# KerkDovan/univer-ocr

Measured on AMD Instinct MI355X. Metric: document-images/sec (fwd+bwd) on 256x512 synthetic pages, higher is better.
Workload: dtype f32; 1 GPU; BASELINE configs[2]: my_model train step (fwd+loss+bwd+L2+SGD) of Monochrome+Paragraph+Line on (32,256,512,1) pages and Char on (32,32,64,1) line strips per GPU; batch_per_gpu=32, global_batch=32, optimizer=sgd, parallelism=dp1, h2d_inclusive=False, input_grads=True, hip_graphs=True, pipelined_lanes=True, hw_queues=4

## Files before the change

### include/univer_hip.h

```cpp
#ifndef UNIVER_HIP_H
#define UNIVER_HIP_H

#include <stddef.h>
#include <stdint.h>

#ifdef __cplusplus
extern "C" {
#endif

#define UOCR_ABI_VERSION 4

typedef struct uocr_ctx uocr_ctx;

enum { UOCR_F32 = 0, UOCR_F64 = 1, UOCR_F16 = 2 };
#define UOCR_F16_SCALED(k) (UOCR_F16 | ((k) << 8))
#define UOCR_DTYPE_BASE(dtype) ((dtype) & 0xff)
#define UOCR_DTYPE_GRAD_SCALE_LOG2(dtype) (((dtype) >> 8) & 0xff)
enum { UOCR_ACT_NONE = 0, UOCR_ACT_RELU = 1, UOCR_ACT_LEAKY = 2, UOCR_ACT_SIGMOID = 3 };
enum { UOCR_LOSS_DICE = 0, UOCR_LOSS_JACCARD = 1 };
enum {
    UOCR_OK = 0,
    UOCR_ERR_ARG = -1,
    UOCR_ERR_DTYPE = -2,
    UOCR_ERR_HIP = -3,
    UOCR_ERR_WORKSPACE = -4,
    UOCR_ERR_UNSUPPORTED = -5,
    UOCR_ERR_RCCL = -6
};

int uocr_abi_version(void);
int uocr_ctx_create(int device, size_t workspace_bytes, uocr_ctx** out);
int uocr_ctx_create_cu_mask(int device, size_t workspace_bytes, const uint32_t* cu_mask, int mask_words, uocr_ctx** out);
int uocr_ctx_destroy(uocr_ctx* ctx);
int uocr_ctx_set_stream(uocr_ctx* ctx, void* hip_stream);
void* uocr_ctx_get_stream(uocr_ctx* ctx);
int uocr_ctx_set_option(uocr_ctx* ctx, const char* key, int value);
int uocr_ctx_last_split(uocr_ctx* ctx, int* blocks, long long* items);
int uocr_ctx_last_gemm(uocr_ctx* ctx, int* bm, int* gm, int* gn, int* nsplit);
int uocr_ctx_last_gemm_group(uocr_ctx* ctx, int* problems, int* split_problems);
int uocr_ctx_last_pair(uocr_ctx* ctx, int* kernel, int* g, int* mode, int* pf, int* nw, int* blocks_x, int* bands,
                       int* band_h);
int uocr_ctx_reserve_workspace(uocr_ctx* ctx, size_t bytes);
const char* uocr_last_error(uocr_ctx* ctx);
int uocr_malloc(uocr_ctx* ctx, size_t bytes, void** out);
int uocr_free(uocr_ctx* ctx, void* ptr);
int uocr_memset_zero(uocr_ctx* ctx, void* ptr, size_t bytes);
int uocr_h2d(uocr_ctx* ctx, void* dst, const void* src_host, size_t bytes);
int uocr_d2h_sync(uocr_ctx* ctx, void* dst_host, const void* src, size_t bytes);
int uocr_d2d(uocr_ctx* ctx, void* dst, const void* src, size_t bytes);
int uocr_stream_sync(uocr_ctx* ctx);
int uocr_event_create(void** out_event);
int uocr_event_destroy(void* event);
int uocr_event_record(uocr_ctx* ctx, void* event);
int uocr_stream_wait_event(uocr_ctx* ctx, void* event);
int uocr_event_elapsed_ms_sync(void* start, void* stop, float* out_ms);
int uocr_event_synchronize(void* event);
int uocr_graph_begin_capture(uocr_ctx* ctx);
int uocr_graph_end_capture(uocr_ctx* ctx, void** out_graph_exec);
int uocr_graph_launch(uocr_ctx* ctx, void* graph_exec);
int uocr_graph_destroy(void* graph_exec);
int uocr_ctx_set_loss_snapshot(uocr_ctx* ctx, const double* slots, int count, double* ring, int ring_len,
                               unsigned* counter);
int uocr_wgrad_defer_begin(uocr_ctx* ctx);
int uocr_wgrad_defer_flush(uocr_ctx* ctx, int keep_open);
int uocr_device_info(uocr_ctx* ctx, char* name_out, size_t name_cap, int* cu_count, size_t* hbm_bytes);

int uocr_conv2d_fwd(uocr_ctx* ctx, int dtype, const void* x, const void* w, const void* b, void* y,
                    int n, int h, int wd, int cin, int cout, int kh, int kw, int sh, int sw,
                    int ph, int pw, int oh, int ow, double pad_value, int use_bias,
                    int act, double act_alpha);
int uocr_conv2d_bwd_data(uocr_ctx* ctx, int dtype, const void* dy, const void* w, void* dx,
                         int n, int h, int wd, int cin, int cout, int kh, int kw, int sh, int sw,
                         int ph, int pw, int oh, int ow,
                         const void* x_act, int act, double act_alpha);
int uocr_conv2d_bwd_weight(uocr_ctx* ctx, int dtype, const void* x, const void* dy, void* dw, void* db,
                           int n, int h, int wd, int cin, int cout, int kh, int kw, int sh, int sw,
                           int ph, int pw, int oh, int ow, double pad_value, int use_bias,
                           int accumulate);

int uocr_conv_pair_fwd(uocr_ctx* ctx, int dtype, const void* x, const void* w1, const void* b1,
                       const void* w2, const void* b2, void* y, int n, int h, int wd, int cmid,
                       double pad_value1, int use_bias1, int use_bias2, double alpha1, int act2);
int uocr_conv_pair_bwd(uocr_ctx* ctx, int dtype, const void* x, const void* y, const void* dy,
                       const void* w1, const void* b1, const void* w2, void* dw1, void* db1, void* dw2,
                       void* db2, void* dx, int n, int h, int wd, int cmid, double pad_value1,
                       int use_bias1, int use_bias2, double alpha1, int act2, int accumulate);

int uocr_upconv2x_fwd(uocr_ctx* ctx, int dtype, const void* x_low, const void* w, const void* b, void* y,
                      int n, int hl, int wl, int cin, int cout, int kh, int kw, int ph, int pw,
                      int use_bias, int act, double act_alpha, void* weff);
int uocr_upconv2x_bwd_data(uocr_ctx* ctx, int dtype, const void* dy, const void* w, void* dx_low,
                           int n, int hl, int wl, int cin, int cout, int kh, int kw, int ph, int pw,
                           const void* x_act, int act, double act_alpha, const void* weff);
int uocr_upconv2x_bwd_weight(uocr_ctx* ctx, int dtype, const void* x_low, const void* dy, void* dw, void* db,
                             int n, int hl, int wl, int cin, int cout, int kh, int kw, int ph, int pw,
                             int use_bias, int accumulate);

int uocr_maxpool2d_fwd(uocr_ctx* ctx, int dtype, const void* x, void* y, uint8_t* mask,
                       int n, int h, int wd, int c, int kh, int kw, int sh, int sw, int ph, int pw,
                       int oh, int ow);
int uocr_maxpool2d_bwd(uocr_ctx* ctx, int dtype, const void* dy, const uint8_t* mask, void* dx,
                       int n, int h, int wd, int c, int kh, int kw, int sh, int sw, int ph, int pw,
                       int oh, int ow);

int uocr_upsample2d_fwd(uocr_ctx* ctx, int dtype, const void* x, void* y,
                        int n, int h, int wd, int c, int sy, int sx);
int uocr_upsample2d_bwd(uocr_ctx* ctx, int dtype, const void* dy, void* dx,
                        int n, int h, int wd, int c, int sy, int sx);

int uocr_act_fwd(uocr_ctx* ctx, int dtype, int kind, double alpha, const void* x, void* y, size_t count);
int uocr_act_bwd(uocr_ctx* ctx, int dtype, int kind, double alpha, const void* x, const void* dy,
                 void* dx, size_t count);

int uocr_act_bwd_from_output(uocr_ctx* ctx, int dtype, int kind, double alpha, const void* y, const void* dy,
                             void* dx, size_t count);

int uocr_dense_fwd(uocr_ctx* ctx, int dtype, const void* x, const void* w, void* y,
                   int m, int n_in, int n_out);
int uocr_dense_bwd(uocr_ctx* ctx, int dtype, const void* x, const void* w, const void* dy,
                   void* dx, void* dw, int m, int n_in, int n_out, int accumulate);
int uocr_dense_fwd_act(uocr_ctx* ctx, int dtype, const void* x, const void* w, void* y,
                       int m, int n_in, int n_out, int act, double act_alpha);
int uocr_dense_bwd_act(uocr_ctx* ctx, int dtype, const void* x, const void* w, const void* dy,
                       void* dx, void* dw, int m, int n_in, int n_out, int accumulate,
                       int x_act, double x_act_alpha);

int uocr_fixed_width_fwd(uocr_ctx* ctx, int dtype, const void* x, void* y,
                         int n, int h, int wd, int c, int width);
int uocr_fixed_width_bwd(uocr_ctx* ctx, int dtype, const void* dy, void* dx,
                         int n, int h, int wd, int c, int width);

int uocr_copy_2d(uocr_ctx* ctx, int dtype, void* dst, size_t dst_ld, const void* src, size_t src_ld,
                 size_t rows, size_t cols);
int uocr_add(uocr_ctx* ctx, int dtype, const void* a, const void* b, void* out, size_t count);
int uocr_axpy(uocr_ctx* ctx, int dtype, double alpha, const void* x, void* y, size_t count);
int uocr_scale(uocr_ctx* ctx, int dtype, double alpha, void* x, size_t count);
int uocr_fill(uocr_ctx* ctx, int dtype, void* x, double value, size_t count);
int uocr_convert(uocr_ctx* ctx, int src_dtype, const void* src, int dst_dtype, void* dst, size_t count);
int uocr_u8_to_float(uocr_ctx* ctx, int dtype, const uint8_t* src, void* dst, double scale, size_t count);

int uocr_seg_loss(uocr_ctx* ctx, int dtype, int kind , const void* pred,
                  const void* gt, void* grad , double* loss_out,
                  int n, int hw, int c, int out_act);
int uocr_softmax_ce(uocr_ctx* ctx, int dtype, const void* pred, const void* gt, void* grad ,
                    double* loss_out, int m, int c);
int uocr_sigmoid_ce(uocr_ctx* ctx, int dtype, const void* pred, const void* gt, void* grad ,
                    double* loss_out, int m, size_t count);

int uocr_l2_reg(uocr_ctx* ctx, int dtype, const void* w, void* grad, size_t count, double strength,
                double* loss_out, int accumulate_loss);
int uocr_l1_reg(uocr_ctx* ctx, int dtype, const void* w, void* grad, size_t count, double strength,
                double* loss_out, int accumulate_loss);

int uocr_adam_step(uocr_ctx* ctx, int dtype, void* w, const void* g, void* v, void* a, size_t count,
                   double lr, double beta1, double beta2, double eps);
int uocr_momentum_step(uocr_ctx* ctx, int dtype, void* w, const void* g, void* v, size_t count,
                       double lr, double momentum);
int uocr_momentum_step_fused(uocr_ctx* ctx, int dtype, void* w, void* g, void* v, size_t count, double lr,
                             double momentum, int nranges, const long long* lo, const long long* hi,
                             const int* kind, const double* strength, double* reg_loss_out, int zero_grad,
                             const double* hyper_dev);
int uocr_adam_step_fused(uocr_ctx* ctx, int dtype, void* w, void* g, void* v, void* a, size_t count, double lr,
                         double beta1, double beta2, double eps, int nranges, const long long* lo,
                         const long long* hi, const int* kind, const double* strength, double* reg_loss_out,
                         int zero_grad, const double* hyper_dev );
int uocr_rmsprop_step(uocr_ctx* ctx, int dtype, void* w, const void* g, void* a, size_t count,
                      double lr, double rho, double eps);
int uocr_has_nan(uocr_ctx* ctx, int dtype, const void* x, size_t count, int32_t* flag_out);

#define UOCR_DP_UNIQUE_ID_BYTES 128
int uocr_dp_get_unique_id(void* out_bytes );
int uocr_dp_init(uocr_ctx* ctx, int rank, int world, const void* unique_id_bytes);
int uocr_dp_info(uocr_ctx* ctx, int* rank, int* world );
int uocr_dp_allreduce_sum(uocr_ctx* ctx, void* buf, size_t count, int dtype);
int uocr_dp_broadcast(uocr_ctx* ctx, void* buf, size_t count, int dtype, int root);
int uocr_dp_finalize(uocr_ctx* ctx);
int uocr_dp_version(int* out_version);

#ifdef __cplusplus
}
#endif
#endif
```

### univer-ocr_amd/csrc/conv_up.hip

```cpp
#include "up_phase.h"
#include "finish_group.h"
#include "conv_dims.h"

namespace {

using f32x4 = __attribute__((ext_vector_type(4))) float;

constexpr int CH = 4;
constexpr int RH = 16, RW = 32;
constexpr int XH = RH + 2, XW = RW + 2;
constexpr int XPLANE = 624;
constexpr int NWEFF = 9 * CH * 16;

__device__ __forceinline__ f32x4 mfma(float a, float b, f32x4 c) {
    return __builtin_amdgcn_mfma_f32_16x16x4f32(a, b, c, 0, 0, 0);
}

__device__ __forceinline__ float act_apply(float v, int act, float alpha) {
    switch (act) {
        case UOCR_ACT_RELU: return v * (v >= 0.f ? 1.f : 0.f);
        case UOCR_ACT_LEAKY: return v * ((v >= 0.f ? 1.f : 0.f) + alpha * (v < 0.f ? 1.f : 0.f));
        case UOCR_ACT_SIGMOID: return 1.f / (1.f + expf(-v));
        default: return v;
    }
}

__host__ __device__ __forceinline__ void tap_group(int phase, int mi, int& lo, int& hi) {
    if (phase == 0) {
        lo = 2 * mi;
        hi = mi == 2 ? 5 : 2 * mi + 2;
    } else {
        lo = mi == 0 ? 0 : 2 * mi - 1;
        hi = mi == 0 ? 1 : 2 * mi + 1;
    }
}

__global__ __launch_bounds__(256) void upconv_weff_kernel(const float* __restrict__ w, float* __restrict__ weff) {
    for (int i = threadIdx.x; i < NWEFF; i += blockDim.x) {
        const int o = i & 3, phase = (i >> 2) & 3, c = (i >> 4) & 3, m = i >> 6;
        int ylo, yhi, xlo, xhi;
        tap_group(phase >> 1, m / 3, ylo, yhi);
        tap_group(phase & 1, m % 3, xlo, xhi);
        float s = 0.f;
        for (int ky = ylo; ky < yhi; ++ky)
            for (int kx = xlo; kx < xhi; ++kx) s += w[((ky * 5 + kx) * CH + c) * CH + o];
        weff[i] = s;
    }
}

template <typename TA>
__device__ __forceinline__ void stage_planar(float* __restrict__ xs, const TA* __restrict__ xb, int ry, int rx,
                                             int hl, int wl, int tid) {
    if constexpr (sizeof(TA) == 4) {
        stage_batched<XH * XW, 256, 3, float4>(
            tid,
            [&](int i, bool& inside) {
                const int r = i / XW, c = i - r * XW;
                const int gy = ry - 1 + r, gx = rx - 1 + c;
                inside = gy >= 0 && gy < hl && gx >= 0 && gx < wl;
                return reinterpret_cast<const float4*>(xb + ((size_t)min(max(gy, 0), hl - 1) * wl + min(max(gx, 0), wl - 1)) * CH);
            },
            [&](int i, float4 v, bool inside) {
                if (!inside) v = make_float4(0.f, 0.f, 0.f, 0.f);
                xs[i] = v.x;
                xs[XPLANE + i] = v.y;
                xs[2 * XPLANE + i] = v.z;
                xs[3 * XPLANE + i] = v.w;
            });
        return;
    }
    for (int i = tid; i < XH * XW; i += 256) {
        const int r = i / XW, c = i - r * XW;
        const int gy = ry - 1 + r, gx = rx - 1 + c;
        float4 v = make_float4(0.f, 0.f, 0.f, 0.f);
        if (gy >= 0 && gy < hl && gx >= 0 && gx < wl) v = ld4(xb + ((size_t)gy * wl + gx) * CH);
        xs[i] = v.x;
        xs[XPLANE + i] = v.y;
        xs[2 * XPLANE + i] = v.z;
        xs[3 * XPLANE + i] = v.w;
    }
}

template <typename TA>
__global__ __launch_bounds__(256) void upconv_fwd_kernel(const TA* __restrict__ xl, const float* __restrict__ w,
                                                         const float* __restrict__ bias, TA* __restrict__ y,
                                                         int hl, int wl, int rows_per_block, int use_bias, int act,
                                                         float alpha, float* __restrict__ weff_out) {
    __shared__ float xs[CH * XPLANE];
    const int tid = threadIdx.x, lane = tid & 63, wv = tid >> 6, n = lane & 15, kq = lane >> 4;
    if (weff_out && blockIdx.x == 0 && blockIdx.y == 0 && blockIdx.z == 0) {
        for (int i = tid; i < NWEFF; i += 256) {
            const int o = i & 3, phase = (i >> 2) & 3, c = (i >> 4) & 3, m = i >> 6;
            int ylo, yhi, xlo, xhi;
            tap_group(phase >> 1, m / 3, ylo, yhi);
            tap_group(phase & 1, m % 3, xlo, xhi);
            float s = 0.f;
            for (int ky = ylo; ky < yhi; ++ky)
                for (int kx = xlo; kx < xhi; ++kx) s += w[((ky * 5 + kx) * CH + c) * CH + o];
            weff_out[i] = s;
        }
    }
    const int rx = blockIdx.x * RW;
    const int row_begin = blockIdx.y * rows_per_block, row_end = min(hl, row_begin + rows_per_block);
    const TA* xb = xl + (size_t)blockIdx.z * hl * wl * CH;
    const int W = 2 * wl;
    TA* yb = y + (size_t)blockIdx.z * (2 * hl) * W * CH;
    float wa[9];
#pragma unroll
    for (int t = 0; t < 9; ++t) {
        int ylo, yhi, xlo, xhi;
        tap_group(n >> 3, t / 3, ylo, yhi);
        tap_group((n >> 2) & 1, t % 3, xlo, xhi);
        float s = 0.f;
        for (int ky = ylo; ky < yhi; ++ky)
            for (int kx = xlo; kx < xhi; ++kx) s += w[((ky * 5 + kx) * CH + kq) * CH + (n & 3)];
        wa[t] = s;
    }
    f32x4 b4 = {0.f, 0.f, 0.f, 0.f};
    if (use_bias) b4 = f32x4{bias[0], bias[1], bias[2], bias[3]};
    for (int ry = row_begin; ry < row_end; ry += RH) {
        __syncthreads();
        stage_planar(xs, xb, ry, rx, hl, wl, tid);
        __syncthreads();
#pragma unroll 2
        for (int k = 0; k < 8; ++k) {
            const int gi = wv * 8 + k, r = gi >> 1, c0 = (gi & 1) * 16;
            const float* xr = xs + kq * XPLANE + r * XW + c0 + n;
            f32x4 acc = b4;
#pragma unroll
            for (int t = 0; t < 9; ++t) acc = mfma(wa[t], xr[(t / 3) * XW + t % 3], acc);
            const int py = ry + r, pxl = rx + c0 + n;
            if (py < row_end && pxl < wl) {
                float4 out;
                out.x = act_apply(acc[0], act, alpha);
                out.y = act_apply(acc[1], act, alpha);
                out.z = act_apply(acc[2], act, alpha);
                out.w = act_apply(acc[3], act, alpha);
                st4(yb + ((size_t)(2 * py + (kq >> 1)) * W + 2 * pxl + (kq & 1)) * CH, out);
            }
        }
    }
}

template <typename TA>
__global__ __launch_bounds__(256) void upconv_wgrad_kernel(const TA* __restrict__ xl, const TA* __restrict__ dy,
                                                           float* __restrict__ partial, int hl, int wl,
                                                           int rows_per_block) {
    __shared__ float xs[CH * XPLANE];
    __shared__ float red[4][48][16];
    __shared__ float reddb[4][64];
    const int tid = threadIdx.x, lane = tid & 63, wv = tid >> 6, n = lane & 15, kq = lane >> 4;
    const int rx = blockIdx.x * RW;
    const int row_begin = blockIdx.y * rows_per_block, row_end = min(hl, row_begin + rows_per_block);
    const TA* xb = xl + (size_t)blockIdx.z * hl * wl * CH;
    const int W = 2 * wl;
    const TA* gb = dy + (size_t)blockIdx.z * (2 * hl) * W * CH;
    int aoff[3];
    bool aok[3];
#pragma unroll
    for (int j = 0; j < 3; ++j) {
        const int K = 16 * j + n;
        aok[j] = K < 36;
        const int Kc = aok[j] ? K : 35, t = Kc >> 2;
        aoff[j] = (Kc & 3) * XPLANE + (t / 3) * XW + t % 3 + kq;
    }
    const int boff = ((n >> 3) * W + ((n >> 2) & 1)) * CH + (n & 3);
    f32x4 acc[3] = {{0.f, 0.f, 0.f, 0.f}, {0.f, 0.f, 0.f, 0.f}, {0.f, 0.f, 0.f, 0.f}};
    float dbacc = 0.f;
    for (int ry = row_begin; ry < row_end; ry += RH) {
        __syncthreads();
        stage_planar(xs, xb, ry, rx, hl, wl, tid);
        __syncthreads();
#pragma unroll 2
        for (int k = 0; k < 8; ++k) {
            const int gi = wv * 8 + k, r = gi >> 1, c0 = (gi & 1) * 16;
            const int py = ry + r;
            const bool row_ok = py < row_end;
            const float* xr = xs + r * XW + c0;
            const TA* gr = gb + ((size_t)(2 * min(py, hl - 1)) * W + 2 * rx) * CH + boff;
#pragma unroll
            for (int i = 0; i < 4; ++i) {
                const int pl = c0 + 4 * i + kq;
                const bool ok = row_ok && rx + pl < wl;
                float g = ld1(gr + (size_t)2 * min(pl, wl - 1 - rx) * CH);
                g = ok ? g : 0.f;
                dbacc += g;
#pragma unroll
                for (int j = 0; j < 3; ++j) {
                    const float xv = xr[4 * i + aoff[j]];
                    acc[j] = mfma(aok[j] ? xv : 0.f, g, acc[j]);
                }
            }
        }
    }
#pragma unroll
    for (int j = 0; j < 3; ++j)
#pragma unroll
        for (int v = 0; v < 4; ++v) red[wv][16 * j + 4 * kq + v][n] = acc[j][v];
    reddb[wv][lane] = dbacc;
    __syncthreads();
    if (tid < 4) {
        float s = 0.f;
        for (int w = 0; w < 4; ++w)
            for (int l = tid; l < 64; l += 4) s += reddb[w][l];
        reddb[0][tid] = s;
    }
    __syncthreads();
    const int blk = (blockIdx.z * gridDim.y + blockIdx.y) * gridDim.x + blockIdx.x;
    up4_write_row(partial + (size_t)blk * UP4_NOUT, [&](int i) {
        if (i >= 576) return reddb[0][i - 576];
        const int K = i >> 4, col = i & 15;
        return red[0][K][col] + red[1][K][col] + red[2][K][col] + red[3][K][col];
    }, tid, 256);
}

__global__ __launch_bounds__(256) void colsum_finish_kernel(const float* __restrict__ partial, int nblocks, int ncols,
                                                            int ndw, float* __restrict__ dw, float* __restrict__ db,
                                                            int use_bias, int accumulate, float unscale) {
    constexpr int FC = 8, NSEG = 32;
    __shared__ double seg[NSEG][FC];
    const int o = threadIdx.x % FC, sg = threadIdx.x / FC, j = blockIdx.x * FC + o;
    double s = 0.0;
    if (j < ncols) {
        const int per = (nblocks + NSEG - 1) / NSEG, b0 = sg * per, b1 = min(nblocks, b0 + per);
        int b = b0;
        for (; b + 8 <= b1; b += 8) {
            float v[8];
#pragma unroll
            for (int k = 0; k < 8; ++k) v[k] = partial[(size_t)(b + k) * ncols + j];
#pragma unroll
            for (int k = 0; k < 8; ++k) s += (double)v[k];
        }
        for (; b < b1; ++b) s += (double)partial[(size_t)b * ncols + j];
    }
    seg[sg][o] = s;
    __syncthreads();
    if (sg != 0 || j >= ncols) return;
#pragma unroll
    for (int k = 1; k < NSEG; ++k) s += seg[k][o];
    float* dst = j < ndw ? dw + j : db + (j - ndw);
    if (j >= ndw && !use_bias) s = 0.0;
    s *= (double)unscale;
    *dst = accumulate ? (float)((double)*dst + s) : (float)s;
}

constexpr int GH = 2 * (RH + 2), GW = 2 * (RW + 2);
template <typename TA>
__global__ __launch_bounds__(256) void upconv_dgrad_kernel(const TA* __restrict__ dy, const float* __restrict__ weff,
                                                           TA* __restrict__ dxl, int hl, int wl,
                                                           const TA* __restrict__ mask_y, int mask_act,
                                                           float mask_alpha) {
    __shared__ float4 gs[GH * GW];
    const int tid = threadIdx.x;
    const int rx = blockIdx.x * RW, ry = blockIdx.y * RH;
    const int H = 2 * hl, W = 2 * wl;
    const TA* gb = dy + (size_t)blockIdx.z * H * W * CH;
    if constexpr (sizeof(TA) == 4) {
        stage_batched<GH * GW, 256, 5, float4>(
            tid,
            [&](int i, bool& inside) {
                const int r = i / GW, c = i - r * GW;
                const int gy = 2 * (ry - 1) + r, gx = 2 * (rx - 1) + c;
                inside = gy >= 0 && gy < H && gx >= 0 && gx < W;
                return reinterpret_cast<const float4*>(gb + ((size_t)min(max(gy, 0), H - 1) * W + min(max(gx, 0), W - 1)) * CH);
            },
            [&](int i, float4 v, bool inside) { gs[i] = inside ? v : make_float4(0.f, 0.f, 0.f, 0.f); });
    } else {
        for (int i = tid; i < GH * GW; i += 256) {
            const int r = i / GW, c = i - r * GW;
            const int gy = 2 * (ry - 1) + r, gx = 2 * (rx - 1) + c;
            float4 v = make_float4(0.f, 0.f, 0.f, 0.f);
            if (gy >= 0 && gy < H && gx >= 0 && gx < W) v = ld4(gb + ((size_t)gy * W + gx) * CH);
            gs[i] = v;
        }
    }
    __syncthreads();
    const int c = tid & 31, r0 = tid >> 5;
    float acc[2][4];
#pragma unroll
    for (int p = 0; p < 2; ++p)
#pragma unroll
        for (int j = 0; j < 4; ++j) acc[p][j] = 0.f;
#pragma unroll 1
    for (int m = 0; m < 9; ++m) {
        const float* wt = weff + m * 64;
        const int my = m / 3 - 1, mx = m % 3 - 1;
#pragma unroll
        for (int p = 0; p < 2; ++p) {
            const int r = r0 + 8 * p;
            const float4* g0 = gs + (2 * (r - my + 1)) * GW + 2 * (c - mx + 1);
            const float4 g[4] = {g0[0], g0[1], g0[GW], g0[GW + 1]};
#pragma unroll
            for (int ch = 0; ch < 4; ++ch)
#pragma unroll
                for (int phase = 0; phase < 4; ++phase) {
                    const float* wv = wt + ch * 16 + phase * 4;
                    acc[p][ch] += wv[0] * g[phase].x + wv[1] * g[phase].y + wv[2] * g[phase].z + wv[3] * g[phase].w;
                }
        }
    }
#pragma unroll
    for (int p = 0; p < 2; ++p) {
        const int qy = ry + r0 + 8 * p, qx = rx + c;
        if (qy >= hl || qx >= wl) continue;
        const size_t off = (((size_t)blockIdx.z * hl + qy) * wl + qx) * CH;
        float4 out = make_float4(acc[p][0], acc[p][1], acc[p][2], acc[p][3]);
        if (mask_act != UOCR_ACT_NONE) {
            const float4 yv = ld4(mask_y + off);
            out.x *= act_grad_from_output<float>(yv.x, mask_act, mask_alpha);
            out.y *= act_grad_from_output<float>(yv.y, mask_act, mask_alpha);
            out.z *= act_grad_from_output<float>(yv.z, mask_act, mask_alpha);
            out.w *= act_grad_from_output<float>(yv.w, mask_act, mask_alpha);
        }
        st4(dxl + off, out);
    }
}

__device__ __forceinline__ void weff1_build(float (&we)[36], const float* __restrict__ w) {
#pragma unroll
    for (int m = 0; m < 9; ++m)
#pragma unroll
        for (int phase = 0; phase < 4; ++phase) {
            int ylo, yhi, xlo, xhi;
            tap_group(phase >> 1, m / 3, ylo, yhi);
            tap_group(phase & 1, m % 3, xlo, xhi);
            float s = 0.f;
            for (int ky = ylo; ky < yhi; ++ky)
                for (int kx = xlo; kx < xhi; ++kx) s += w[ky * 5 + kx];
            we[m * 4 + phase] = s;
        }
}

template <typename TA>
__global__ __launch_bounds__(256) void up1_fwd_kernel(const TA* __restrict__ xl, const float* __restrict__ w,
                                                      const float* __restrict__ bias, TA* __restrict__ y, int hl,
                                                      int wl, int use_bias, int act, float alpha) {
    __shared__ float xs[XH * XW];
    const int tid = threadIdx.x;
    const int rx = blockIdx.x * RW, ry = blockIdx.y * RH;
    const TA* xb = xl + (size_t)blockIdx.z * hl * wl;
    stage_batched<XH * XW, 256, 3, TA>(
        tid,
        [&](int i, bool& inside) {
            const int r = i / XW, c = i - r * XW;
            const int gy = ry - 1 + r, gx = rx - 1 + c;
            inside = gy >= 0 && gy < hl && gx >= 0 && gx < wl;
            return xb + (size_t)min(max(gy, 0), hl - 1) * wl + min(max(gx, 0), wl - 1);
        },
        [&](int i, TA v, bool inside) { xs[i] = inside ? (float)v : 0.f; });
    float we[36];
    weff1_build(we, w);
    const float b0 = use_bias ? bias[0] : 0.f;
    __syncthreads();
    const int c = tid & 31, r0 = tid >> 5;
    const int W = 2 * wl;
    TA* yb = y + (size_t)blockIdx.z * (2 * hl) * W;
#pragma unroll
    for (int p = 0; p < 2; ++p) {
        const int r = r0 + 8 * p, py = ry + r, pxl = rx + c;
        float acc[4] = {b0, b0, b0, b0};
#pragma unroll
        for (int m = 0; m < 9; ++m) {
            const float xv = xs[(r + m / 3) * XW + c + m % 3];
#pragma unroll
            for (int phase = 0; phase < 4; ++phase) acc[phase] += xv * we[m * 4 + phase];
        }
        if (py < hl && pxl < wl) {
            TA* o = yb + (size_t)(2 * py) * W + 2 * pxl;
            st2(o, make_float2(act_apply(acc[0], act, alpha), act_apply(acc[1], act, alpha)));
            st2(o + W, make_float2(act_apply(acc[2], act, alpha), act_apply(acc[3], act, alpha)));
        }
    }
}

template <typename TA>
__global__ __launch_bounds__(256) void up1_dgrad_kernel(const TA* __restrict__ dy, const float* __restrict__ w,
                                                        TA* __restrict__ dxl, int hl, int wl,
                                                        const TA* __restrict__ mask_y, int mask_act,
                                                        float mask_alpha) {
    __shared__ float gs[GH * GW];
    const int tid = threadIdx.x;
    const int rx = blockIdx.x * RW, ry = blockIdx.y * RH;
    const int H = 2 * hl, W = 2 * wl;
    const TA* gb = dy + (size_t)blockIdx.z * H * W;
    stage_batched<GH * GW, 256, 10, TA>(
        tid,
        [&](int i, bool& inside) {
            const int r = i / GW, c = i - r * GW;
            const int gy = 2 * (ry - 1) + r, gx = 2 * (rx - 1) + c;
            inside = gy >= 0 && gy < H && gx >= 0 && gx < W;
            return gb + (size_t)min(max(gy, 0), H - 1) * W + min(max(gx, 0), W - 1);
        },
        [&](int i, TA v, bool inside) { gs[i] = inside ? (float)v : 0.f; });
    float we[36];
    weff1_build(we, w);
    __syncthreads();
    const int c = tid & 31, r0 = tid >> 5;
#pragma unroll
    for (int p = 0; p < 2; ++p) {
        const int r = r0 + 8 * p;
        float acc = 0.f;
#pragma unroll
        for (int m = 0; m < 9; ++m) {
            const int my = m / 3 - 1, mx = m % 3 - 1;
            const float* g0 = gs + (2 * (r - my + 1)) * GW + 2 * (c - mx + 1);
            acc += we[m * 4] * g0[0] + we[m * 4 + 1] * g0[1] + we[m * 4 + 2] * g0[GW] + we[m * 4 + 3] * g0[GW + 1];
        }
        const int qy = ry + r, qx = rx + c;
        if (qy >= hl || qx >= wl) continue;
        const size_t off = ((size_t)blockIdx.z * hl + qy) * wl + qx;
        if (mask_act != UOCR_ACT_NONE) acc *= act_grad_from_output<float>(ld1(mask_y + off), mask_act, mask_alpha);
        st1(dxl + off, acc);
    }
}

template <typename TA>
__global__ __launch_bounds__(256) void up1_wgrad_kernel(const TA* __restrict__ xl, const TA* __restrict__ dy,
                                                        float* __restrict__ partial, int hl, int wl,
                                                        int rows_per_block) {
    __shared__ float xs[XH * XW];
    __shared__ float red[4][37];
    const int tid = threadIdx.x;
    const int rx = blockIdx.x * RW;
    const int row_begin = blockIdx.y * rows_per_block, row_end = min(hl, row_begin + rows_per_block);
    const TA* xb = xl + (size_t)blockIdx.z * hl * wl;
    const int W = 2 * wl;
    const TA* gb = dy + (size_t)blockIdx.z * (2 * hl) * W;
    const int c = tid & 31, r0 = tid >> 5;
    float acc[36], dbacc = 0.f;
#pragma unroll
    for (int i = 0; i < 36; ++i) acc[i] = 0.f;
    for (int ry = row_begin; ry < row_end; ry += RH) {
        __syncthreads();
        stage_batched<XH * XW, 256, 3, TA>(
            tid,
            [&](int i, bool& inside) {
                const int r = i / XW, cc = i - r * XW;
                const int gy = ry - 1 + r, gx = rx - 1 + cc;
                inside = gy >= 0 && gy < hl && gx >= 0 && gx < wl;
                return xb + (size_t)min(max(gy, 0), hl - 1) * wl + min(max(gx, 0), wl - 1);
            },
            [&](int i, TA v, bool inside) { xs[i] = inside ? (float)v : 0.f; });
        __syncthreads();
#pragma unroll
        for (int p = 0; p < 2; ++p) {
            const int r = r0 + 8 * p, py = ry + r, pxl = rx + c;
            if (py >= row_end || pxl >= wl) continue;
            const TA* g0 = gb + (size_t)(2 * py) * W + 2 * pxl;
            const float2 ga = ld2(g0), gbv = ld2(g0 + W);
            const float g[4] = {ga.x, ga.y, gbv.x, gbv.y};
            dbacc += (g[0] + g[1]) + (g[2] + g[3]);
#pragma unroll
            for (int m = 0; m < 9; ++m) {
                const float xv = xs[(r + m / 3) * XW + c + m % 3];
#pragma unroll
                for (int phase = 0; phase < 4; ++phase) acc[m * 4 + phase] += xv * g[phase];
            }
        }
    }
    const int lane = tid & 63, wv = tid >> 6;
#pragma unroll
    for (int i = 0; i < 36; ++i) {
        const float v = wave_reduce_sum(acc[i]);
        if (lane == 0) red[wv][i] = v;
    }
    dbacc = wave_reduce_sum(dbacc);
    if (lane == 0) red[wv][36] = dbacc;
    __syncthreads();
    const int blk = (blockIdx.z * gridDim.y + blockIdx.y) * gridDim.x + blockIdx.x;
    up1_write_row(partial + (size_t)blk * UP1_NOUT, [&](int i) { return red[0][i] + red[1][i] + red[2][i] + red[3][i]; }, tid);
}


int up_rows_per_block(int strips, int hl, int n, unsigned max_blocks = 2048u) {
    int rows = RH;
    while (rows < hl && (size_t)strips * ((hl + rows - 1) / rows) * n > max_blocks) rows += RH;
    return rows;
}

int check_up(uocr_ctx* ctx, int dtype, int n, int hl, int wl, int cin, int cout, int kh, int kw, int ph, int pw) {
    if (UOCR_DTYPE_BASE(dtype) != UOCR_F32 && UOCR_DTYPE_BASE(dtype) != UOCR_F16)
        UOCR_FAIL(ctx, UOCR_ERR_UNSUPPORTED, "upconv2x: float32 / float16 only");
    if (!((cin == CH && cout == CH) || (cin == 1 && cout == 1)) || kh != 5 || kw != 5 || ph != 2 || pw != 2)
        UOCR_FAIL(ctx, UOCR_ERR_UNSUPPORTED,
                  "upconv2x: 5x5 / padding 2 / 4 -> 4 or 1 -> 1 channels only (got %dx%d pad %d,%d %d -> %d)", kh, kw, ph,
                  pw, cin, cout);
    UOCR_REQUIRE(ctx, n > 0 && hl > 0 && wl > 0 && n <= 65535);
    return UOCR_OK;
}

}

extern "C" int uocr_upconv2x_fwd(uocr_ctx* ctx, int dtype, const void* x_low, const void* w, const void* b, void* y,
                                 int n, int hl, int wl, int cin, int cout, int kh, int kw, int ph, int pw,
                                 int use_bias, int act, double act_alpha, void* weff) {
    UOCR_CHECK_CTX(ctx);
    UOCR_REQUIRE(ctx, x_low && w && b && y);
    int rc = check_up(ctx, dtype, n, hl, wl, cin, cout, kh, kw, ph, pw);
    if (rc != UOCR_OK) return rc;
    if (uocr_upconv_h16_eligible(ctx, dtype, cin, cout) && uocr_aligned_act(x_low, dtype) && uocr_aligned_act(y, dtype))
        return uocr_upconv_fwd_h16(ctx, x_low, w, b, y, n, hl, wl, use_bias, act, act_alpha);
    const int strips = (wl + RW - 1) / RW, rows = up_rows_per_block(strips, hl, n, (unsigned)uocr_budget(ctx, 2048));
    if (cin != 1) uocr_note_split(ctx, (long long)strips * ((hl + rows - 1) / rows) * n, (long long)strips * ((hl + RH - 1) / RH) * n);
    UOCR_DISPATCH_TA(ctx, dtype, {
        if (cin == 1)
            hipLaunchKernelGGL((up1_fwd_kernel<TA>), dim3((wl + RW - 1) / RW, (hl + RH - 1) / RH, n), dim3(256), 0,
                               ctx->stream, (const TA*)x_low, (const float*)w, (const float*)b, (TA*)y, hl, wl, use_bias,
                               act, (float)act_alpha);
        else
            hipLaunchKernelGGL((upconv_fwd_kernel<TA>), dim3(strips, (hl + rows - 1) / rows, n), dim3(256), 0,
                               ctx->stream, (const TA*)x_low, (const float*)w, (const float*)b, (TA*)y, hl, wl, rows,
                               use_bias, act, (float)act_alpha, (float*)weff);
    });
    UOCR_LAUNCH_CHECK(ctx);
    return UOCR_OK;
}

extern "C" int uocr_upconv2x_bwd_data(uocr_ctx* ctx, int dtype, const void* dy, const void* w, void* dx_low, int n,
                                      int hl, int wl, int cin, int cout, int kh, int kw, int ph, int pw,
                                      const void* x_act, int act, double act_alpha, const void* weff_in) {
    UOCR_CHECK_CTX(ctx);
    UOCR_REQUIRE(ctx, dy && w && dx_low);
    UOCR_REQUIRE(ctx, act == UOCR_ACT_NONE || x_act != nullptr);
    int rc = check_up(ctx, dtype, n, hl, wl, cin, cout, kh, kw, ph, pw);
    if (rc != UOCR_OK) return rc;
    if (uocr_upconv_h16_eligible(ctx, dtype, cin, cout) && uocr_aligned_act(dy, dtype) &&
        uocr_aligned_act(dx_low, dtype) && (act == UOCR_ACT_NONE || uocr_aligned_act(x_act, dtype)))
        return uocr_upconv_dgrad_h16(ctx, dy, w, dx_low, n, hl, wl, act == UOCR_ACT_NONE ? nullptr : x_act, act, act_alpha);
    if (uocr_upconv_t32_eligible(ctx, dtype, cin, cout) && (reinterpret_cast<uintptr_t>(dy) & 15u) == 0 &&
        (reinterpret_cast<uintptr_t>(dx_low) & 15u) == 0 && (act == UOCR_ACT_NONE || (reinterpret_cast<uintptr_t>(x_act) & 15u) == 0))
        return uocr_upconv_dgrad_t32(ctx, dy, w, dx_low, n, hl, wl, cin, act == UOCR_ACT_NONE ? nullptr : x_act, act, act_alpha);
    const float* weff = (const float*)weff_in;
    if (cin != 1 && !weff) {
        rc = uocr_need_workspace(ctx, NWEFF * sizeof(float));
        if (rc != UOCR_OK) return rc;
        hipLaunchKernelGGL(upconv_weff_kernel, dim3(1), dim3(256), 0, ctx->stream, (const float*)w, (float*)ctx->workspace);
        weff = (const float*)ctx->workspace;
    }
    const dim3 grid((wl + RW - 1) / RW, (hl + RH - 1) / RH, n);
    UOCR_DISPATCH_TA(ctx, dtype, {
        if (cin == 1)
            hipLaunchKernelGGL((up1_dgrad_kernel<TA>), grid, dim3(256), 0, ctx->stream, (const TA*)dy, (const float*)w,
                               (TA*)dx_low, hl, wl, (const TA*)x_act, act, (float)act_alpha);
        else
            hipLaunchKernelGGL((upconv_dgrad_kernel<TA>), grid, dim3(256), 0, ctx->stream, (const TA*)dy,
                               weff, (TA*)dx_low, hl, wl, (const TA*)x_act, act, (float)act_alpha);
    });
    UOCR_LAUNCH_CHECK(ctx);
    return UOCR_OK;
}

extern "C" int uocr_upconv2x_bwd_weight(uocr_ctx* ctx, int dtype, const void* x_low, const void* dy, void* dw, void* db,
                                        int n, int hl, int wl, int cin, int cout, int kh, int kw, int ph, int pw,
                                        int use_bias, int accumulate) {
    UOCR_CHECK_CTX(ctx);
    UOCR_REQUIRE(ctx, x_low && dy && dw && db);
    int rc = check_up(ctx, dtype, n, hl, wl, cin, cout, kh, kw, ph, pw);
    if (rc != UOCR_OK) return rc;
    const float unscale = (float)uocr_grad_unscale(dtype);
    const int ncols = cin == 1 ? UP1_NOUT : UP4_NOUT, ndw = ncols - cin;
    auto finish = [&](const float* partial, int nblocks) -> int {
        FinishDesc fd{};
        fd.kind = FIN_COLS;
        fd.partial = partial;
        fd.nblocks = nblocks;
        fd.ncols = fd.group_cols = ncols;
        fd.row_stride = ncols;
        fd.dw = (float*)dw, fd.db = (float*)db;
        fd.use_bias = use_bias, fd.accumulate = accumulate;
        fd.unscale = unscale;
        fd.p[0] = ndw;
        if (uocr_finish_defer(ctx, fd)) return UOCR_OK;
        hipLaunchKernelGGL(colsum_finish_kernel, dim3((ncols + 7) / 8), dim3(256), 0, ctx->stream, partial, nblocks, ncols,
                           ndw, (float*)dw, (float*)db, use_bias, accumulate, unscale);
        UOCR_LAUNCH_CHECK(ctx);
        return UOCR_OK;
    };
    if (UOCR_DTYPE_BASE(dtype) == UOCR_F16 && ctx->opt_fast && ctx->opt_h16 && uocr_aligned_act(x_low, dtype) &&
        uocr_aligned_act(dy, dtype)) {
        const size_t floats = (size_t)ctx->cu_count * 8 * ncols;
        float* partial = uocr_partial_buffer(ctx, floats * sizeof(float), &rc);
        if (rc != UOCR_OK) return rc;
        int nblocks = 0;
        rc = uocr_upconv_wgrad_h16(ctx, x_low, dy, partial, floats, n, hl, wl, cin, &nblocks);
        if (rc != UOCR_OK) return rc;
        return finish(partial, nblocks);
    }
    const int strips = (wl + RW - 1) / RW, rows = up_rows_per_block(strips, hl, n, (unsigned)uocr_budget(ctx, 1024));
    const int bands = (hl + rows - 1) / rows, nblocks = strips * bands * n;
    uocr_note_split(ctx, nblocks, (long long)strips * ((hl + RH - 1) / RH) * n);
    float* partial = uocr_partial_buffer(ctx, (size_t)nblocks * ncols * sizeof(float), &rc);
    if (rc != UOCR_OK) return rc;
    UOCR_DISPATCH_TA(ctx, dtype, {
        if (cin == 1)
            hipLaunchKernelGGL((up1_wgrad_kernel<TA>), dim3(strips, bands, n), dim3(256), 0, ctx->stream,
                               (const TA*)x_low, (const TA*)dy, partial, hl, wl, rows);
        else
            hipLaunchKernelGGL((upconv_wgrad_kernel<TA>), dim3(strips, bands, n), dim3(256), 0, ctx->stream,
                               (const TA*)x_low, (const TA*)dy, partial, hl, wl, rows);
    });
    UOCR_LAUNCH_CHECK(ctx);
    return finish(partial, nblocks);
}
```

### univer-ocr_amd/csrc/ctx.hip

```cpp
#include <cstdlib>

#include "finish_group.h"
#include "gemm.h"
#include "uocr_common.h"

extern "C" {

int uocr_abi_version(void) { return UOCR_ABI_VERSION; }

int uocr_ctx_create(int device, size_t workspace_bytes, uocr_ctx** out) {
    if (!out || device < 0) return UOCR_ERR_ARG;
    *out = nullptr;
    int count = 0;
    if (hipGetDeviceCount(&count) != hipSuccess || device >= count) return UOCR_ERR_HIP;
    if (hipSetDevice(device) != hipSuccess) return UOCR_ERR_HIP;
    uocr_ctx* ctx = new uocr_ctx();
    ctx->device = device;
    ctx->err[0] = 0;
    ctx->workspace = nullptr;
    ctx->workspace_bytes = 0;
    ctx->sync = nullptr;
    ctx->gemm_defer = nullptr;
    ctx->snap_src = nullptr;
    ctx->snap_count = 0;
    ctx->snap_ring = nullptr;
    ctx->snap_ring_len = 0;
    ctx->snap_counter = nullptr;
    ctx->finish_defer = nullptr;
    ctx->owns_stream = true;
    ctx->opt_mfma = 1;
    ctx->opt_fast = 1;
    ctx->opt_tiled = 1;
    ctx->opt_split = 1024;
    ctx->opt_split_min = 3;
    ctx->opt_bm = 0;
    ctx->opt_h16 = 1;
    ctx->opt_t32 = 2;
    ctx->opt_xcd = 1;
    ctx->opt_pair_band = 0;
    ctx->opt_pair_g = 4;
    ctx->opt_group_blocks = 0;
    ctx->opt_wgrad_bands = 0;
    ctx->opt_max_blocks = 0;
    ctx->split_blocks = 0;
    ctx->split_items = 0;
    ctx->gemm_bm = ctx->gemm_gm = ctx->gemm_gn = ctx->gemm_nsplit = 0;
    ctx->gemm_group_count = ctx->gemm_group_split = 0;
    uocr_note_pair(ctx, 0, 0, 0, 0, 0, 0, 0, 0);
    ctx->opt_h3 = 0;
#ifdef UOCR_EXPERIMENTS
    if (const char* e = getenv("UOCR_H3")) ctx->opt_h3 = atoi(e);
#endif
    ctx->opt_pair_pf = -1;
    if (const char* e = getenv("UOCR_PAIR_PF")) ctx->opt_pair_pf = atoi(e);
    if (const char* e = getenv("UOCR_WGRAD_BANDS")) ctx->opt_wgrad_bands = atoi(e);
    if (hipStreamCreateWithFlags(&ctx->stream, hipStreamNonBlocking) != hipSuccess) {
        delete ctx;
        return UOCR_ERR_HIP;
    }
    hipDeviceProp_t prop;
    ctx->cu_count = 256;
    if (hipGetDeviceProperties(&prop, device) == hipSuccess) ctx->cu_count = prop.multiProcessorCount;
    if (workspace_bytes) {
        if (hipMalloc(&ctx->workspace, workspace_bytes) != hipSuccess) {
            hipStreamDestroy(ctx->stream);
            delete ctx;
            return UOCR_ERR_HIP;
        }
        ctx->workspace_bytes = workspace_bytes;
    }
    if (hipMalloc((void**)&ctx->sync, UOCR_SYNC_WORDS * sizeof(unsigned)) != hipSuccess ||
        hipMemsetAsync(ctx->sync, 0, UOCR_SYNC_WORDS * sizeof(unsigned), ctx->stream) != hipSuccess ||
        hipStreamSynchronize(ctx->stream) != hipSuccess) {
        if (ctx->sync) hipFree(ctx->sync);
        if (ctx->workspace) hipFree(ctx->workspace);
        hipStreamDestroy(ctx->stream);
        delete ctx;
        return UOCR_ERR_HIP;
    }
    *out = ctx;
    return UOCR_OK;
}

int uocr_ctx_create_cu_mask(int device, size_t workspace_bytes, const uint32_t* cu_mask, int mask_words, uocr_ctx** out) {
    if (!out || !cu_mask || mask_words <= 0) return UOCR_ERR_ARG;
    int rc = uocr_ctx_create(device, workspace_bytes, out);
    if (rc != UOCR_OK) return rc;
    uocr_ctx* ctx = *out;
    hipStream_t masked = nullptr;
    if (hipExtStreamCreateWithCUMask(&masked, (uint32_t)mask_words, cu_mask) != hipSuccess) {
        uocr_ctx_destroy(ctx);
        *out = nullptr;
        return UOCR_ERR_HIP;
    }
    hipStreamDestroy(ctx->stream);
    ctx->stream = masked;
    int cus = 0;
    for (int i = 0; i < mask_words; ++i) cus += __builtin_popcount(cu_mask[i]);
    if (cus > 0 && cus < ctx->cu_count) ctx->cu_count = cus;
    return UOCR_OK;
}

int uocr_ctx_destroy(uocr_ctx* ctx) {
    UOCR_CHECK_CTX(ctx);
    hipSetDevice(ctx->device);
    hipStreamSynchronize(ctx->stream);
    if (ctx->workspace) hipFree(ctx->workspace);
    if (ctx->sync) hipFree(ctx->sync);
    uocr_gemm_defer_free(ctx);
    uocr_finish_defer_free(ctx);
    if (ctx->owns_stream) hipStreamDestroy(ctx->stream);
    delete ctx;
    return UOCR_OK;
}

int uocr_ctx_set_stream(uocr_ctx* ctx, void* hip_stream) {
    UOCR_CHECK_CTX(ctx);
    if (ctx->owns_stream) {
        UOCR_HIP(ctx, hipStreamSynchronize(ctx->stream));
        UOCR_HIP(ctx, hipStreamDestroy(ctx->stream));
        ctx->owns_stream = false;
    }
    ctx->stream = (hipStream_t)hip_stream;
    return UOCR_OK;
}

int uocr_ctx_set_option(uocr_ctx* ctx, const char* key, int value) {
    UOCR_CHECK_CTX(ctx);
    UOCR_REQUIRE(ctx, key != nullptr);
    if (!strcmp(key, "mfma")) ctx->opt_mfma = value;
    else if (!strcmp(key, "fast_paths")) ctx->opt_fast = value;
    else if (!strcmp(key, "tiled")) ctx->opt_tiled = value;
    else if (!strcmp(key, "split_blocks")) ctx->opt_split = value;
    else if (!strcmp(key, "split_min")) ctx->opt_split_min = value;
    else if (!strcmp(key, "gemm_bm")) ctx->opt_bm = value;
    else if (!strcmp(key, "xcd_remap")) ctx->opt_xcd = value;
    else if (!strcmp(key, "h16")) ctx->opt_h16 = value;
    else if (!strcmp(key, "t32")) {
        if (value & ~UOCR_T32_BUILT)
            UOCR_FAIL(ctx, UOCR_ERR_UNSUPPORTED, "option t32 = %d asks for kernels this library was built without "
                      "(UOCR_BUILD_EXPERIMENTS=1 ./build.sh)", value);
        ctx->opt_t32 = value;
    }
    else if (!strcmp(key, "pair_band")) ctx->opt_pair_band = value;
    else if (!strcmp(key, "pair_g")) ctx->opt_pair_g = value;
    else if (!strcmp(key, "group_blocks")) ctx->opt_group_blocks = value;
    else if (!strcmp(key, "wgrad_bands") && value >= 0) ctx->opt_wgrad_bands = value;
    else if (!strcmp(key, "max_blocks") && value >= 0) ctx->opt_max_blocks = value;
    else if (!strcmp(key, "h3")) {
#ifndef UOCR_EXPERIMENTS
        if (value) UOCR_FAIL(ctx, UOCR_ERR_UNSUPPORTED, "option h3: this library was built without conv_h3 "
                             "(UOCR_BUILD_EXPERIMENTS=1 ./build.sh)");
#endif
        ctx->opt_h3 = value;
    }
    else if (!strcmp(key, "pair_pf")) ctx->opt_pair_pf = value;
    else UOCR_FAIL(ctx, UOCR_ERR_ARG, "unknown option '%s'", key);
    return UOCR_OK;
}

int uocr_ctx_last_split(uocr_ctx* ctx, int* blocks, long long* items) {
    UOCR_CHECK_CTX(ctx);
    UOCR_REQUIRE(ctx, blocks && items);
    *blocks = ctx->split_blocks;
    *items = ctx->split_items;
    return UOCR_OK;
}

int uocr_ctx_last_gemm(uocr_ctx* ctx, int* bm, int* gm, int* gn, int* nsplit) {
    UOCR_CHECK_CTX(ctx);
    UOCR_REQUIRE(ctx, bm && gm && gn && nsplit);
    *bm = ctx->gemm_bm;
    *gm = ctx->gemm_gm;
    *gn = ctx->gemm_gn;
    *nsplit = ctx->gemm_nsplit;
    return UOCR_OK;
}

int uocr_ctx_last_gemm_group(uocr_ctx* ctx, int* problems, int* split_problems) {
    UOCR_CHECK_CTX(ctx);
    UOCR_REQUIRE(ctx, problems && split_problems);
    *problems = ctx->gemm_group_count;
    *split_problems = ctx->gemm_group_split;
    return UOCR_OK;
}

int uocr_ctx_last_pair(uocr_ctx* ctx, int* kernel, int* g, int* mode, int* pf, int* nw, int* blocks_x, int* bands,
                       int* band_h) {
    UOCR_CHECK_CTX(ctx);
    UOCR_REQUIRE(ctx, kernel && g && mode && pf && nw && blocks_x && bands && band_h);
    *kernel = ctx->pair_kernel;
    *g = ctx->pair_g;
    *mode = ctx->pair_mode;
    *pf = ctx->pair_pf;
    *nw = ctx->pair_nw;
    *blocks_x = ctx->pair_blocks_x;
    *bands = ctx->pair_bands;
    *band_h = ctx->pair_band_h;
    return UOCR_OK;
}

void* uocr_ctx_get_stream(uocr_ctx* ctx) { return ctx ? (void*)ctx->stream : nullptr; }

int uocr_ctx_reserve_workspace(uocr_ctx* ctx, size_t bytes) {
    UOCR_CHECK_CTX(ctx);
    if (bytes <= ctx->workspace_bytes) return UOCR_OK;
    UOCR_HIP(ctx, hipSetDevice(ctx->device));
    UOCR_HIP(ctx, hipStreamSynchronize(ctx->stream));
    if (ctx->workspace) UOCR_HIP(ctx, hipFree(ctx->workspace));
    ctx->workspace = nullptr;
    ctx->workspace_bytes = 0;
    UOCR_HIP(ctx, hipMalloc(&ctx->workspace, bytes));
    ctx->workspace_bytes = bytes;
    return UOCR_OK;
}

const char* uocr_last_error(uocr_ctx* ctx) { return ctx ? ctx->err : "null context"; }

int uocr_malloc(uocr_ctx* ctx, size_t bytes, void** out) {
    UOCR_CHECK_CTX(ctx);
    UOCR_REQUIRE(ctx, out != nullptr);
    UOCR_HIP(ctx, hipSetDevice(ctx->device));
    UOCR_HIP(ctx, hipMalloc(out, bytes ? bytes : 1));
    return UOCR_OK;
}

int uocr_free(uocr_ctx* ctx, void* ptr) {
    UOCR_CHECK_CTX(ctx);
    if (ptr) UOCR_HIP(ctx, hipFree(ptr));
    return UOCR_OK;
}

int uocr_memset_zero(uocr_ctx* ctx, void* ptr, size_t bytes) {
    UOCR_CHECK_CTX(ctx);
    if (!bytes) return UOCR_OK;
    UOCR_REQUIRE(ctx, ptr != nullptr);
    UOCR_HIP(ctx, hipMemsetAsync(ptr, 0, bytes, ctx->stream));
    return UOCR_OK;
}

int uocr_h2d(uocr_ctx* ctx, void* dst, const void* src_host, size_t bytes) {
    UOCR_CHECK_CTX(ctx);
    if (!bytes) return UOCR_OK;
    UOCR_REQUIRE(ctx, dst && src_host);
    UOCR_HIP(ctx, hipMemcpyAsync(dst, src_host, bytes, hipMemcpyHostToDevice, ctx->stream));
    return UOCR_OK;
}

int uocr_d2h_sync(uocr_ctx* ctx, void* dst_host, const void* src, size_t bytes) {
    UOCR_CHECK_CTX(ctx);
    if (!bytes) return UOCR_OK;
    UOCR_REQUIRE(ctx, dst_host && src);
    UOCR_HIP(ctx, hipMemcpyAsync(dst_host, src, bytes, hipMemcpyDeviceToHost, ctx->stream));
    UOCR_HIP(ctx, hipStreamSynchronize(ctx->stream));
    return UOCR_OK;
}

int uocr_d2d(uocr_ctx* ctx, void* dst, const void* src, size_t bytes) {
    UOCR_CHECK_CTX(ctx);
    if (!bytes) return UOCR_OK;
    UOCR_REQUIRE(ctx, dst && src);
    UOCR_HIP(ctx, hipMemcpyAsync(dst, src, bytes, hipMemcpyDeviceToDevice, ctx->stream));
    return UOCR_OK;
}

int uocr_stream_sync(uocr_ctx* ctx) {
    UOCR_CHECK_CTX(ctx);
    UOCR_HIP(ctx, hipStreamSynchronize(ctx->stream));
    return UOCR_OK;
}

int uocr_event_create(void** out_event) {
    if (!out_event) return UOCR_ERR_ARG;
    hipEvent_t ev;
    if (hipEventCreate(&ev) != hipSuccess) return UOCR_ERR_HIP;
    *out_event = (void*)ev;
    return UOCR_OK;
}

int uocr_event_destroy(void* event) {
    if (!event) return UOCR_ERR_ARG;
    return hipEventDestroy((hipEvent_t)event) == hipSuccess ? UOCR_OK : UOCR_ERR_HIP;
}

int uocr_event_record(uocr_ctx* ctx, void* event) {
    UOCR_CHECK_CTX(ctx);
    UOCR_REQUIRE(ctx, event != nullptr);
    UOCR_HIP(ctx, hipEventRecord((hipEvent_t)event, ctx->stream));
    return UOCR_OK;
}

int uocr_stream_wait_event(uocr_ctx* ctx, void* event) {
    UOCR_CHECK_CTX(ctx);
    UOCR_REQUIRE(ctx, event != nullptr);
    UOCR_HIP(ctx, hipStreamWaitEvent(ctx->stream, (hipEvent_t)event, 0));
    return UOCR_OK;
}

int uocr_event_elapsed_ms_sync(void* start, void* stop, float* out_ms) {
    if (!start || !stop || !out_ms) return UOCR_ERR_ARG;
    if (hipEventSynchronize((hipEvent_t)stop) != hipSuccess) return UOCR_ERR_HIP;
    return hipEventElapsedTime(out_ms, (hipEvent_t)start, (hipEvent_t)stop) == hipSuccess ? UOCR_OK
                                                                                           : UOCR_ERR_HIP;
}

int uocr_event_synchronize(void* event) {
    if (!event) return UOCR_ERR_ARG;
    return hipEventSynchronize((hipEvent_t)event) == hipSuccess ? UOCR_OK : UOCR_ERR_HIP;
}

int uocr_graph_begin_capture(uocr_ctx* ctx) {
    UOCR_CHECK_CTX(ctx);
    UOCR_HIP(ctx, hipStreamBeginCapture(ctx->stream, hipStreamCaptureModeRelaxed));
    return UOCR_OK;
}

int uocr_graph_end_capture(uocr_ctx* ctx, void** out_graph_exec) {
    UOCR_CHECK_CTX(ctx);
    UOCR_REQUIRE(ctx, out_graph_exec != nullptr);
    *out_graph_exec = nullptr;
    hipGraph_t graph = nullptr;
    UOCR_HIP(ctx, hipStreamEndCapture(ctx->stream, &graph));
    hipGraphExec_t exec = nullptr;
    const hipError_t e = hipGraphInstantiate(&exec, graph, nullptr, nullptr, 0);
    hipGraphDestroy(graph);
    if (e != hipSuccess) UOCR_FAIL(ctx, UOCR_ERR_HIP, "hipGraphInstantiate failed: %s", hipGetErrorString(e));
    *out_graph_exec = (void*)exec;
    return UOCR_OK;
}

int uocr_graph_launch(uocr_ctx* ctx, void* graph_exec) {
    UOCR_CHECK_CTX(ctx);
    UOCR_REQUIRE(ctx, graph_exec != nullptr);
    UOCR_HIP(ctx, hipGraphLaunch((hipGraphExec_t)graph_exec, ctx->stream));
    return UOCR_OK;
}

int uocr_graph_destroy(void* graph_exec) {
    if (!graph_exec) return UOCR_ERR_ARG;
    return hipGraphExecDestroy((hipGraphExec_t)graph_exec) == hipSuccess ? UOCR_OK : UOCR_ERR_HIP;
}

int uocr_device_info(uocr_ctx* ctx, char* name_out, size_t name_cap, int* cu_count, size_t* hbm_bytes) {
    UOCR_CHECK_CTX(ctx);
    hipDeviceProp_t prop;
    UOCR_HIP(ctx, hipGetDeviceProperties(&prop, ctx->device));
    if (name_out && name_cap) {
        strncpy(name_out, prop.name, name_cap - 1);
        name_out[name_cap - 1] = 0;
    }
    if (cu_count) *cu_count = prop.multiProcessorCount;
    if (hbm_bytes) *hbm_bytes = prop.totalGlobalMem;
    return UOCR_OK;
}

}
```

### univer-ocr_amd/csrc/uocr_common.h

```cpp
#pragma once
#include <hip/hip_runtime.h>
#include <stdint.h>
#include <stdio.h>
#include <string.h>

#include "univer_hip.h"

struct uocr_ctx {
    int device;
    hipStream_t stream;
    bool owns_stream;
    void* workspace;
    size_t workspace_bytes;
    const double* snap_src;
    int snap_count;
    double* snap_ring;
    int snap_ring_len;
    unsigned* snap_counter;
    void* gemm_defer;
    void* finish_defer;
    unsigned* sync;
    int cu_count;
    int opt_mfma;
    int opt_fast;
    int opt_tiled;
    int opt_split;
    int opt_split_min;
    int opt_xcd;
    int opt_bm;
    int opt_h16;
    int opt_t32;
    int opt_pair_band;
    int opt_pair_pf;
    int opt_h3;
    int opt_group_blocks;
    int opt_wgrad_bands;
    int opt_pair_g;
    int opt_max_blocks;
    int split_blocks;
    long long split_items;
    int gemm_bm, gemm_gm, gemm_gn, gemm_nsplit;
    int gemm_group_count, gemm_group_split;
    int pair_kernel, pair_g, pair_mode, pair_pf;
    int pair_nw, pair_blocks_x, pair_bands, pair_band_h;
    char err[512];
};

constexpr int UOCR_SYNC_WORDS = 1 << 18;
#ifdef UOCR_EXPERIMENTS
constexpr int UOCR_T32_BUILT = 255;
#else
constexpr int UOCR_T32_BUILT = 2;
#endif

#define UOCR_FAIL(ctx, code, ...)                                   \
    do {                                                            \
        if (ctx) snprintf((ctx)->err, sizeof((ctx)->err), __VA_ARGS__); \
        return (code);                                              \
    } while (0)

#define UOCR_HIP(ctx, call)                                                              \
    do {                                                                                 \
        hipError_t e_ = (call);                                                          \
        if (e_ != hipSuccess)                                                            \
            UOCR_FAIL(ctx, UOCR_ERR_HIP, "%s failed: %s (%s:%d)", #call, hipGetErrorString(e_), \
                      __FILE__, __LINE__);                                               \
    } while (0)

#define UOCR_LAUNCH_CHECK(ctx)                                                           \
    do {                                                                                 \
        hipError_t e_ = hipGetLastError();                                               \
        if (e_ != hipSuccess)                                                            \
            UOCR_FAIL(ctx, UOCR_ERR_HIP, "kernel launch failed: %s (%s:%d)", hipGetErrorString(e_), \
                      __FILE__, __LINE__);                                               \
    } while (0)

#define UOCR_REQUIRE(ctx, cond)                                                          \
    do {                                                                                 \
        if (!(cond)) UOCR_FAIL(ctx, UOCR_ERR_ARG, "bad argument: %s (%s:%d)", #cond, __FILE__, __LINE__); \
    } while (0)

#define UOCR_CHECK_CTX(ctx) \
    do {                    \
        if (!(ctx)) return UOCR_ERR_ARG; \
    } while (0)

#define UOCR_DISPATCH(ctx, dtype, ...)                                   \
    do {                                                                 \
        if ((dtype) == UOCR_F32) { using T = float; __VA_ARGS__; }       \
        else if ((dtype) == UOCR_F64) { using T = double; __VA_ARGS__; } \
        else UOCR_FAIL(ctx, UOCR_ERR_DTYPE, "unknown dtype %d", (int)(dtype)); \
    } while (0)

#define UOCR_DISPATCH_ACT(ctx, dtype, ...)                                                        \
    do {                                                                                          \
        const int base_ = UOCR_DTYPE_BASE(dtype);                                                 \
        if (base_ == UOCR_F32) { using TS = float; using T = float; __VA_ARGS__; }                \
        else if (base_ == UOCR_F64) { using TS = double; using T = double; __VA_ARGS__; }         \
        else if (base_ == UOCR_F16) { using TS = _Float16; using T = float; __VA_ARGS__; }        \
        else UOCR_FAIL(ctx, UOCR_ERR_DTYPE, "unknown dtype %d", (int)(dtype));                    \
    } while (0)

#define UOCR_DISPATCH_STORAGE(ctx, dtype, ...)                                                    \
    do {                                                                                          \
        const int base_ = UOCR_DTYPE_BASE(dtype);                                                 \
        if (base_ == UOCR_F32) { using T = float; __VA_ARGS__; }                                  \
        else if (base_ == UOCR_F64) { using T = double; __VA_ARGS__; }                            \
        else if (base_ == UOCR_F16) { using T = _Float16; __VA_ARGS__; }                          \
        else UOCR_FAIL(ctx, UOCR_ERR_DTYPE, "unknown dtype %d", (int)(dtype));                    \
    } while (0)

static inline double uocr_grad_scale(int dtype) {
    return UOCR_DTYPE_BASE(dtype) == UOCR_F16 ? (double)(1u << (UOCR_DTYPE_GRAD_SCALE_LOG2(dtype) & 31)) : 1.0;
}
static inline double uocr_grad_unscale(int dtype) { return 1.0 / uocr_grad_scale(dtype); }

static inline int uocr_need_workspace(uocr_ctx* ctx, size_t bytes) {
    if (bytes > ctx->workspace_bytes)
        UOCR_FAIL(ctx, UOCR_ERR_WORKSPACE, "workspace too small: need %zu bytes, have %zu", bytes,
                  ctx->workspace_bytes);
    return UOCR_OK;
}

static inline unsigned uocr_blocks_for(size_t items, unsigned per_block, unsigned cap) {
    size_t b = (items + per_block - 1) / per_block;
    if (b < 1) b = 1;
    if (b > cap) b = cap;
    return (unsigned)b;
}

static inline long uocr_budget(const uocr_ctx* ctx, long budget) {
    return ctx->opt_max_blocks > 0 && ctx->opt_max_blocks < budget ? ctx->opt_max_blocks : budget;
}
static inline void uocr_note_split(uocr_ctx* ctx, long long blocks, long long items) {
    ctx->split_blocks = (int)blocks;
    ctx->split_items = items;
}

static inline void uocr_note_pair(uocr_ctx* ctx, int kernel, int g, int mode, int pf, int nw, int blocks_x, int bands,
                                  int band_h) {
    ctx->pair_kernel = kernel, ctx->pair_g = g, ctx->pair_mode = mode, ctx->pair_pf = pf;
    ctx->pair_nw = nw, ctx->pair_blocks_x = blocks_x, ctx->pair_bands = bands, ctx->pair_band_h = band_h;
}

constexpr unsigned UOCR_MAX_GRID = 2048;
constexpr int UOCR_WAVE = 64;

template <typename T>
__device__ __forceinline__ T wave_reduce_sum(T v) {
#pragma unroll
    for (int off = 32; off > 0; off >>= 1) v += __shfl_down(v, off, 64);
    return v;
}

template <typename T>
__device__ __forceinline__ T wave_reduce_max(T v) {
#pragma unroll
    for (int off = 32; off > 0; off >>= 1) {
        T o = __shfl_down(v, off, 64);
        v = o > v ? o : v;
    }
    return v;
}

__device__ __forceinline__ double block_reduce_sum(double v, double* smem ) {
    const int lane = threadIdx.x & 63, wid = threadIdx.x >> 6;
    v = wave_reduce_sum(v);
    __syncthreads();
    if (lane == 0) smem[wid] = v;
    __syncthreads();
    const int nw = (blockDim.x + 63) >> 6;
    v = (threadIdx.x < (unsigned)nw) ? smem[threadIdx.x] : 0.0;
    if (wid == 0) v = wave_reduce_sum(v);
    return v;
}

__device__ __forceinline__ void pub_store(double* p, double v) {
    __hip_atomic_store(p, v, __ATOMIC_RELAXED, __HIP_MEMORY_SCOPE_AGENT);
}
__device__ __forceinline__ double pub_load(const double* p) {
    return __hip_atomic_load(p, __ATOMIC_RELAXED, __HIP_MEMORY_SCOPE_AGENT);
}
__device__ __forceinline__ unsigned sync_arrive(unsigned* c) {
    asm volatile("s_waitcnt vmcnt(0)" ::: "memory");
    return __hip_atomic_fetch_add(c, 1u, __ATOMIC_RELAXED, __HIP_MEMORY_SCOPE_AGENT);
}
__device__ __forceinline__ unsigned sync_peek(unsigned* c) {
    return __hip_atomic_load(c, __ATOMIC_RELAXED, __HIP_MEMORY_SCOPE_AGENT);
}
__device__ __forceinline__ void sync_clear(unsigned* c) {
    __hip_atomic_store(c, 0u, __ATOMIC_RELAXED, __HIP_MEMORY_SCOPE_AGENT);
}
__device__ __forceinline__ void last_block_sum(unsigned* counter, double* partial, double mine, int count, double scale,
                                               double* out, double* smem ) {
    if (threadIdx.x == 0) {
        pub_store(partial + blockIdx.x, mine);
        const unsigned t = sync_arrive(counter);
        smem[16] = t == gridDim.x - 1 ? 1.0 : 0.0;
    }
    __syncthreads();
    if (smem[16] == 0.0) return;
    double acc = 0.0;
    if (count <= 4 * (int)blockDim.x) {
        double t[4];
#pragma unroll
        for (int k = 0; k < 4; ++k) {
            const int i = threadIdx.x + k * blockDim.x;
            t[k] = i < count ? pub_load(partial + i) : 0.0;
        }
#pragma unroll
        for (int k = 0; k < 4; ++k) acc += t[k];
    } else {
        for (int i = threadIdx.x; i < count; i += blockDim.x) acc += pub_load(partial + i);
    }
    acc = block_reduce_sum(acc, smem);
    if (threadIdx.x == 0) {
        *out = scale * acc;
        sync_clear(counter);
    }
}

using uocr_h2 = __attribute__((ext_vector_type(2))) _Float16;
using uocr_h4 = __attribute__((ext_vector_type(4))) _Float16;

__device__ __forceinline__ float ld1(const float* p) { return *p; }
__device__ __forceinline__ float ld1(const _Float16* p) { return (float)*p; }
__device__ __forceinline__ float2 ld2(const float* p) { return *reinterpret_cast<const float2*>(p); }
__device__ __forceinline__ float2 ld2(const _Float16* p) {
    const uocr_h2 v = *reinterpret_cast<const uocr_h2*>(p);
    return make_float2((float)v.x, (float)v.y);
}
__device__ __forceinline__ float4 ld4(const float* p) { return *reinterpret_cast<const float4*>(p); }
__device__ __forceinline__ float4 ld4(const _Float16* p) {
    const uocr_h4 v = *reinterpret_cast<const uocr_h4*>(p);
    return make_float4((float)v.x, (float)v.y, (float)v.z, (float)v.w);
}
__device__ __forceinline__ void st1(float* p, float v) { *p = v; }
__device__ __forceinline__ void st1(_Float16* p, float v) { *p = (_Float16)v; }
__device__ __forceinline__ void st2(float* p, float2 v) { *reinterpret_cast<float2*>(p) = v; }
__device__ __forceinline__ void st2(_Float16* p, float2 v) {
    uocr_h2 h;
    h.x = (_Float16)v.x;
    h.y = (_Float16)v.y;
    *reinterpret_cast<uocr_h2*>(p) = h;
}
__device__ __forceinline__ void st4(float* p, float4 v) { *reinterpret_cast<float4*>(p) = v; }
__device__ __forceinline__ void st4(_Float16* p, float4 v) {
    uocr_h4 h;
    h.x = (_Float16)v.x;
    h.y = (_Float16)v.y;
    h.z = (_Float16)v.z;
    h.w = (_Float16)v.w;
    *reinterpret_cast<uocr_h4*>(p) = h;
}

#define UOCR_DISPATCH_TA(ctx, dtype, ...)                                                          \
    do {                                                                                           \
        const int base_ = UOCR_DTYPE_BASE(dtype);                                                  \
        if (base_ == UOCR_F32) { using TA = float; __VA_ARGS__; }                                  \
        else if (base_ == UOCR_F16) { using TA = _Float16; __VA_ARGS__; }                          \
        else UOCR_FAIL(ctx, UOCR_ERR_DTYPE, "dtype %d: this kernel exists for float32 / float16 only", (int)(dtype)); \
    } while (0)

static inline bool uocr_aligned_act(const void* p, int dtype) {
    return (reinterpret_cast<uintptr_t>(p) & (UOCR_DTYPE_BASE(dtype) == UOCR_F16 ? 7u : 15u)) == 0;
}

template <typename T>
__device__ __forceinline__ T act_grad_from_output(T y, int act, T alpha) {
    if (act == UOCR_ACT_LEAKY) return y >= T(0) ? T(1) : alpha;
    if (act == UOCR_ACT_SIGMOID) return y * (T(1) - y);
    return T(1);
}

template <int COUNT, int NT, int BATCH, typename V, typename Addr, typename Put>
__device__ __forceinline__ void stage_batched(int tid, Addr addr, Put put) {
    constexpr int K = (COUNT + NT - 1) / NT;
#pragma unroll
    for (int k0 = 0; k0 < K; k0 += BATCH) {
        V v[BATCH];
        bool in[BATCH];
#pragma unroll
        for (int k = 0; k < BATCH; ++k)
            if (k0 + k < K) v[k] = *addr(min(tid + NT * (k0 + k), COUNT - 1), in[k]);
#pragma unroll
        for (int k = 0; k < BATCH; ++k)
            if (k0 + k < K) {
                const int i = tid + NT * (k0 + k);
                if (i < COUNT) put(i, v[k], in[k]);
            }
    }
}

struct TileWalk {
    int strip, trow, img;
    int qx, qy, qz;
    __device__ __forceinline__ TileWalk(int first, int step, int tiles_x, int tiles_y) {
        strip = first % tiles_x;
        int r = first / tiles_x;
        trow = r % tiles_y;
        img = r / tiles_y;
        qx = step % tiles_x;
        r = step / tiles_x;
        qy = r % tiles_y;
        qz = r / tiles_y;
    }
    __device__ __forceinline__ void next(int tiles_x, int tiles_y) {
        strip += qx;
        int carry = strip >= tiles_x;
        strip -= carry ? tiles_x : 0;
        trow += qy + carry;
        carry = trow >= tiles_y;
        trow -= carry ? tiles_y : 0;
        img += qz + carry;
    }
};

int uocr_finish_sum(uocr_ctx* ctx, const double* partial, int count, double scale, double* out, int accumulate);
```

### univer-ocr_amd/hip/lib.py

```python
import ctypes as C
import os

_HERE = os.path.dirname(os.path.abspath(__file__))
_LIB_NAME = 'libuniver_hip.so'

F32, F64, F16 = 0, 1, 2
DP_UNIQUE_ID_BYTES = 128


def f16_scaled(k):
    return F16 | (int(k) << 8)
ACT_NONE, ACT_RELU, ACT_LEAKY, ACT_SIGMOID = 0, 1, 2, 3
LOSS_DICE, LOSS_JACCARD = 0, 1


class HipError(RuntimeError):
    pass


def lib_path():
    return os.path.join(os.path.dirname(_HERE), _LIB_NAME)


def dtype_code(np_dtype):
    import numpy as np
    dt = np.dtype(np_dtype)
    if dt == np.float32:
        return F32
    if dt == np.float64:
        return F64
    if dt == np.float16:
        return F16
    raise HipError(f'unsupported dtype {dt}: the HIP backend stores float16 / float32 / float64')


_vp, _i, _d, _sz = C.c_void_p, C.c_int, C.c_double, C.c_size_t
_ctx = C.c_void_p

_PROTOS = {
    'uocr_ctx_create': [_i, _sz, C.POINTER(_ctx)],
    'uocr_ctx_create_cu_mask': [_i, _sz, C.POINTER(C.c_uint32), _i, C.POINTER(_ctx)],
    'uocr_ctx_destroy': [_ctx],
    'uocr_ctx_set_stream': [_ctx, _vp],
    'uocr_ctx_reserve_workspace': [_ctx, _sz],
    'uocr_ctx_set_option': [_ctx, C.c_char_p, _i],
    'uocr_ctx_last_split': [_ctx, C.POINTER(_i), C.POINTER(C.c_longlong)],
    'uocr_ctx_last_gemm': [_ctx, C.POINTER(_i), C.POINTER(_i), C.POINTER(_i), C.POINTER(_i)],
    'uocr_ctx_last_gemm_group': [_ctx, C.POINTER(_i), C.POINTER(_i)],
    'uocr_ctx_last_pair': [_ctx] + [C.POINTER(_i)] * 8,
    'uocr_malloc': [_ctx, _sz, C.POINTER(_vp)],
    'uocr_free': [_ctx, _vp],
    'uocr_memset_zero': [_ctx, _vp, _sz],
    'uocr_h2d': [_ctx, _vp, _vp, _sz],
    'uocr_d2h_sync': [_ctx, _vp, _vp, _sz],
    'uocr_d2d': [_ctx, _vp, _vp, _sz],
    'uocr_stream_sync': [_ctx],
    'uocr_event_create': [C.POINTER(_vp)],
    'uocr_event_destroy': [_vp],
    'uocr_event_record': [_ctx, _vp],
    'uocr_stream_wait_event': [_ctx, _vp],
    'uocr_event_elapsed_ms_sync': [_vp, _vp, C.POINTER(C.c_float)],
    'uocr_event_synchronize': [_vp],
    'uocr_graph_begin_capture': [_ctx],
    'uocr_graph_end_capture': [_ctx, C.POINTER(_vp)],
    'uocr_graph_launch': [_ctx, _vp],
    'uocr_graph_destroy': [_vp],
    'uocr_ctx_set_loss_snapshot': [_ctx, _vp, _i, _vp, _i, _vp],
    'uocr_wgrad_defer_begin': [_ctx],
    'uocr_wgrad_defer_flush': [_ctx, _i],
    'uocr_device_info': [_ctx, C.c_char_p, _sz, C.POINTER(_i), C.POINTER(_sz)],
    'uocr_conv2d_fwd': [_ctx, _i, _vp, _vp, _vp, _vp] + [_i] * 13 + [_d, _i, _i, _d],
    'uocr_conv2d_bwd_data': [_ctx, _i, _vp, _vp, _vp] + [_i] * 13 + [_vp, _i, _d],
    'uocr_conv2d_bwd_weight': [_ctx, _i, _vp, _vp, _vp, _vp] + [_i] * 13 + [_d, _i, _i],
    'uocr_conv_pair_fwd': [_ctx, _i] + [_vp] * 6 + [_i] * 4 + [_d, _i, _i, _d, _i],
    'uocr_conv_pair_bwd': [_ctx, _i] + [_vp] * 11 + [_i] * 4 + [_d, _i, _i, _d, _i, _i],
    'uocr_upconv2x_fwd': [_ctx, _i, _vp, _vp, _vp, _vp] + [_i] * 9 + [_i, _i, _d, _vp],
    'uocr_upconv2x_bwd_data': [_ctx, _i, _vp, _vp, _vp] + [_i] * 9 + [_vp, _i, _d, _vp],
    'uocr_upconv2x_bwd_weight': [_ctx, _i, _vp, _vp, _vp, _vp] + [_i] * 9 + [_i, _i],
    'uocr_maxpool2d_fwd': [_ctx, _i, _vp, _vp, _vp] + [_i] * 12,
    'uocr_maxpool2d_bwd': [_ctx, _i, _vp, _vp, _vp] + [_i] * 12,
    'uocr_upsample2d_fwd': [_ctx, _i, _vp, _vp] + [_i] * 6,
    'uocr_upsample2d_bwd': [_ctx, _i, _vp, _vp] + [_i] * 6,
    'uocr_act_fwd': [_ctx, _i, _i, _d, _vp, _vp, _sz],
    'uocr_act_bwd': [_ctx, _i, _i, _d, _vp, _vp, _vp, _sz],
    'uocr_act_bwd_from_output': [_ctx, _i, _i, _d, _vp, _vp, _vp, _sz],
    'uocr_dense_fwd': [_ctx, _i, _vp, _vp, _vp, _i, _i, _i],
    'uocr_dense_bwd': [_ctx, _i, _vp, _vp, _vp, _vp, _vp, _i, _i, _i, _i],
    'uocr_dense_fwd_act': [_ctx, _i, _vp, _vp, _vp, _i, _i, _i, _i, _d],
    'uocr_dense_bwd_act': [_ctx, _i, _vp, _vp, _vp, _vp, _vp, _i, _i, _i, _i, _i, _d],
    'uocr_fixed_width_fwd': [_ctx, _i, _vp, _vp] + [_i] * 5,
    'uocr_fixed_width_bwd': [_ctx, _i, _vp, _vp] + [_i] * 5,
    'uocr_copy_2d': [_ctx, _i, _vp, _sz, _vp, _sz, _sz, _sz],
    'uocr_add': [_ctx, _i, _vp, _vp, _vp, _sz],
    'uocr_axpy': [_ctx, _i, _d, _vp, _vp, _sz],
    'uocr_scale': [_ctx, _i, _d, _vp, _sz],
    'uocr_fill': [_ctx, _i, _vp, _d, _sz],
    'uocr_convert': [_ctx, _i, _vp, _i, _vp, _sz],
    'uocr_u8_to_float': [_ctx, _i, _vp, _vp, _d, _sz],
    'uocr_seg_loss': [_ctx, _i, _i, _vp, _vp, _vp, _vp, _i, _i, _i, _i],
    'uocr_softmax_ce': [_ctx, _i, _vp, _vp, _vp, _vp, _i, _i],
    'uocr_sigmoid_ce': [_ctx, _i, _vp, _vp, _vp, _vp, _i, _sz],
    'uocr_l2_reg': [_ctx, _i, _vp, _vp, _sz, _d, _vp, _i],
    'uocr_l1_reg': [_ctx, _i, _vp, _vp, _sz, _d, _vp, _i],
    'uocr_adam_step': [_ctx, _i, _vp, _vp, _vp, _vp, _sz, _d, _d, _d, _d],
    'uocr_momentum_step': [_ctx, _i, _vp, _vp, _vp, _sz, _d, _d],
    'uocr_momentum_step_fused': [_ctx, _i, _vp, _vp, _vp, _sz, _d, _d, _i, C.POINTER(C.c_longlong), C.POINTER(C.c_longlong),
                                 C.POINTER(C.c_int), C.POINTER(C.c_double), _vp, _i, _vp],
    'uocr_adam_step_fused': [_ctx, _i, _vp, _vp, _vp, _vp, _sz, _d, _d, _d, _d, _i, C.POINTER(C.c_longlong),
                             C.POINTER(C.c_longlong), C.POINTER(C.c_int), C.POINTER(C.c_double), _vp, _i, _vp],
    'uocr_rmsprop_step': [_ctx, _i, _vp, _vp, _vp, _sz, _d, _d, _d],
    'uocr_has_nan': [_ctx, _i, _vp, _sz, _vp],
    'uocr_dp_init': [_ctx, _i, _i, _vp],
    'uocr_dp_info': [_ctx, C.POINTER(_i), C.POINTER(_i)],
    'uocr_dp_allreduce_sum': [_ctx, _vp, _sz, _i],
    'uocr_dp_broadcast': [_ctx, _vp, _sz, _i, _i],
    'uocr_dp_finalize': [_ctx],
}
_SPECIAL = {
    'uocr_abi_version': (C.c_int, []),
    'uocr_dp_get_unique_id': (C.c_int, [_vp]),
    'uocr_dp_version': (C.c_int, [C.POINTER(C.c_int)]),
    'uocr_last_error': (C.c_char_p, [_ctx]),
    'uocr_ctx_get_stream': (C.c_void_p, [_ctx]),
}

ABI_SYMBOLS = sorted(list(_PROTOS) + list(_SPECIAL))

_lib = None


def get_lib():
    global _lib
    if _lib is not None:
        return _lib
    path = lib_path()
    if not os.path.exists(path):
        raise HipError(
            f'{path} not found: build it with ./build.sh (or __graft_entry__.build()); '
            f'the HIP backend has no host fallback')
    try:
        import torch
    except ImportError:
        pass
    lib = C.CDLL(path)
    for name, argtypes in _PROTOS.items():
        fn = getattr(lib, name)
        fn.restype = C.c_int
        fn.argtypes = argtypes
    for name, (restype, argtypes) in _SPECIAL.items():
        fn = getattr(lib, name)
        fn.restype = restype
        fn.argtypes = argtypes
    _lib = lib
    return lib
```

### univer-ocr_amd/nn/layers/convolutional.py

```python
import numpy as np

from .. import ops
from ..gpu import CP
from ..help_func import make_list_if_not, tuplize
from ..progress_tracker import track_method
from .layers import BaseLayer, BaseLayerGPU, Param


class Convolutional2D(BaseLayerGPU):
    def __init__(self, kernel_size, in_channels=None, out_channels=None, padding=0, padding_value=0,
                 stride=1, w=None, b=None, bias=True, *args, **kwargs):
        super().__init__(*args, **kwargs)
        self.kernel_size = tuplize('kernel_size', kernel_size, 2)
        self.in_channels, self.out_channels = in_channels, out_channels
        self.padding = tuplize('padding', padding, 2)
        self.padding_value = padding_value
        self.stride = tuplize('stride', stride, 2)
        self.w, self.b, self.bias = w, b, bias
        self.fused_activation = None
        if self.input_shapes is None and in_channels is not None:
            self.input_shapes = [(None, None, None, in_channels)]
        if self.input_shapes is not None:
            self.initialize(self.input_shapes)
        else:
            self.is_initialized = False

    def initialize(self, input_shapes):
        self.input_shapes = input_shapes
        self.in_channels = input_shapes[0][3]
        if self.out_channels is None:
            self.out_channels = self.in_channels
        kh, kw = self.kernel_size
        w_shape = (kh, kw, self.in_channels, self.out_channels)
        b_shape = (self.out_channels,)
        wb = self.initializer(kh * kw * self.in_channels + 1, self.out_channels)
        w = wb[:-1, :].reshape(w_shape) if self.w is None else self.w
        b = wb[-1, :].reshape(b_shape) if self.b is None else self.b
        w = w.value if isinstance(w, Param) else w
        b = b.value if isinstance(b, Param) else b
        assert tuple(w.shape) == w_shape, f'{tuple(w.shape)} != {w_shape}'
        assert tuple(b.shape) == b_shape, f'{tuple(b.shape)} != {b_shape}'
        self.w = Param(w, optimizer=self.optimizer)
        self.b = Param(b, optimizer=self.optimizer)
        self._init_optimizer()
        self.is_initialized = True

    def _forward(self, X, mem_id=0):
        assert X.shape[3] == self.in_channels
        self._mem[mem_id] = X
        return ops.conv2d_fwd(X, self.w.value, self.b.value, self.stride, self.padding, self.padding_value,
                              self.bias)

    def _backward(self, grad, mem_id=0):
        X = self._mem[mem_id]
        ops.conv2d_bwd_weight(X, grad, self.w.grad, self.b.grad, self.stride, self.padding, self.padding_value,
                              self.bias, accumulate=True)
        if not self.needs_input_grad:
            return None
        return ops.conv2d_bwd_data(grad, self.w.value, X.shape, self.stride, self.padding)

    @track_method('forward')
    def forward_fused(self, inputs, activation):
        X = ops.as_device(make_list_if_not(inputs)[0])
        assert X.shape[3] == self.in_channels
        self._mem[0] = X
        y = ops.conv2d_fwd(X, self.w.value, self.b.value, self.stride, self.padding, self.padding_value,
                           self.bias, act=activation.kind, alpha=activation.alpha)
        self._fused_out = y
        return [y]

    @track_method('backward')
    def backward_fused(self, grads, activation=None, act_grad_applied=False, input_activation=None):
        grad = ops.as_device(make_list_if_not(grads)[0])
        if activation is not None and not act_grad_applied:
            grad = ops.act_bwd_from_output(activation.kind, self._fused_out, grad, activation.alpha)
        X = self._mem[0]
        ops.conv2d_bwd_weight(X, grad, self.w.grad, self.b.grad, self.stride, self.padding, self.padding_value,
                              self.bias, accumulate=True)
        if not self.needs_input_grad:
            dx = None
        elif input_activation is None:
            dx = ops.conv2d_bwd_data(grad, self.w.value, X.shape, self.stride, self.padding)
        else:
            dx = ops.conv2d_bwd_data(grad, self.w.value, X.shape, self.stride, self.padding, x_act=X,
                                     act=input_activation.kind, alpha=input_activation.alpha)
        self._fused_out = None
        self.clear_memory()
        return [dx]

    @track_method('forward')
    def forward_up(self, x_low, activation=None):
        x_low = ops.as_device(x_low)
        assert x_low.shape[3] == self.in_channels
        self._mem[0] = x_low
        self._weff = None
        if self.in_channels == 4 and x_low.dtype == np.float32:
            if getattr(self, '_weff_buf', None) is None:
                self._weff_buf = CP.empty((576,), np.float32)
            self._weff = self._weff_buf
        y = ops.upconv2x_fwd(x_low, self.w.value, self.b.value, self.padding, self.bias,
                             None if activation is None else activation.kind,
                             0.0 if activation is None else activation.alpha, weff=self._weff)
        self._fused_out = y if activation is not None else None
        return y

    @track_method('backward')
    def backward_up(self, grads, activation=None, act_grad_applied=False, input_activation=None):
        grad = ops.as_device(make_list_if_not(grads)[0])
        if activation is not None and not act_grad_applied:
            grad = ops.act_bwd_from_output(activation.kind, self._fused_out, grad, activation.alpha)
        x_low = self._mem[0]
        ops.upconv2x_bwd_weight(x_low, grad, self.w.grad, self.b.grad, self.padding, self.bias, accumulate=True)
        weff = getattr(self, '_weff', None)
        self._weff = None
        if input_activation is None:
            dx = ops.upconv2x_bwd_data(grad, self.w.value, x_low.shape, self.padding, weff=weff)
        else:
            dx = ops.upconv2x_bwd_data(grad, self.w.value, x_low.shape, self.padding, x_act=x_low,
                                       act=input_activation.kind, alpha=input_activation.alpha, weff=weff)
        self._fused_out = None
        self.clear_memory()
        return dx

    @track_method('forward')
    def forward_pair(self, X, first, activation, out_activation):
        X = ops.as_device(X)
        first._mem[0] = X
        y = ops.conv_pair_fwd(X, first.w.value, first.b.value, self.w.value, self.b.value, first.padding_value,
                              first.bias, self.bias, activation.alpha,
                              ops.ACT_CODES[None if out_activation is None else out_activation.kind])
        self._fused_out = y
        return y

    @track_method('backward')
    def backward_pair(self, grads, first, activation, out_activation):
        grad = ops.as_device(make_list_if_not(grads)[0])
        X = first._mem[0]
        dx = ops.conv_pair_bwd(X, self._fused_out, grad, first.w.value, first.b.value, self.w.value,
                               first.w.grad, first.b.grad, self.w.grad, self.b.grad, first.padding_value,
                               first.bias, self.bias, activation.alpha,
                               ops.ACT_CODES[None if out_activation is None else out_activation.kind],
                               need_dx=first.needs_input_grad, accumulate=True)
        self._fused_out = None
        first.clear_memory()
        self.clear_memory()
        return dx

    def get_output_shapes(self, input_shapes):
        batch, height, width, _ = make_list_if_not(input_shapes)[0]
        oh, ow = ops.conv_out_hw(height, width, self.kernel_size, self.stride, self.padding)
        return [(batch, oh, ow, self.out_channels)]

    def changes_receptive_field(self):
        return True

    def _get_receptive_field(self, axis, position, output_id):
        assert 0 <= axis < 2, f'Convolutional2D has two axis, found {axis}'
        assert output_id < self.get_outputs_count(), f'This layer has only {self.get_outputs_count()} outputs'
        key = (axis, position, output_id)
        if key not in self._receptive_fields:
            start = position * self.stride[axis] - self.padding[axis]
            self._receptive_fields[key] = {0: set(range(start, start + self.kernel_size[axis]))}
        return self._receptive_fields[key]

    def params(self):
        return {'w': self.w, 'b': self.b}


class Conv2DToBatchedFixedWidthed(BaseLayer):

    def __init__(self, width, *args, **kwargs):
        super().__init__(*args, **kwargs)
        self.width = width

    def _forward(self, X, mem_id=0):
        self.get_output_shapes(X.shape)
        self._mem[mem_id] = X.shape
        return ops.fixed_width_fwd(X, self.width)

    def _backward(self, grad, mem_id=0):
        return ops.fixed_width_bwd(grad, self._mem[mem_id], self.width)

    def get_output_shapes(self, input_shapes):
        result = []
        for bs, h, w, ch in make_list_if_not(input_shapes):
            assert w >= self.width, f'Input width must be >= than output width, found: {w} < {self.width}'
            result.append((bs * w, h, self.width, ch))
        return result
```

### univer-ocr_amd/nn/ops.py

```python
import math

import numpy as np

from ..hip import lib as hiplib
from ..hip.lib import HipError
from .gpu import CP, DeviceArray, DeviceScalar

ACT_CODES = {None: hiplib.ACT_NONE, 'relu': hiplib.ACT_RELU, 'leaky': hiplib.ACT_LEAKY,
             'sigmoid': hiplib.ACT_SIGMOID}


def _rt():
    return CP.runtime()


def _same_dtype(*arrays, grad=None):
    base = arrays[0].code & 0xff
    for a in arrays[1:]:
        other = a.code & 0xff
        if other != base and not (base == hiplib.F16 and other == hiplib.F32):
            raise HipError('mixed dtypes in one op: ' + ', '.join(str(x.dtype) for x in arrays))
    if base == hiplib.F16 and grad is not None:
        return hiplib.f16_scaled(grad.gscale)
    return base


def _like_grad(array, dy):
    array.gscale = dy.gscale
    return array


def f16_grad_scale_log2(kind, n):
    if CP.f16_grad_scale_log2 is not None:
        return int(CP.f16_grad_scale_log2)
    k = int(math.floor(math.log2(max(1, n)))) - (4 if kind == 'seg' else 1)
    return max(0, min(24, k))


def as_device(x):
    if isinstance(x, DeviceArray):
        return x
    return CP.copy(x)


def conv_out_hw(h, w, ks, stride, padding):
    oh = math.floor((h + 2 * padding[0] - (ks[0] - 1) - 1) / stride[0] + 1)
    ow = math.floor((w + 2 * padding[1] - (ks[1] - 1) - 1) / stride[1] + 1)
    return oh, ow


def _conv_dims(x_shape, w_shape, stride, padding):
    n, h, wd, cin = x_shape
    kh, kw, wcin, cout = w_shape
    if cin != wcin:
        raise AssertionError(f'channels mismatch: input has {cin}, weights expect {wcin}')
    oh, ow = conv_out_hw(h, wd, (kh, kw), stride, padding)
    if oh <= 0 or ow <= 0:
        raise HipError(f'convolution output is empty for input {x_shape}, kernel {(kh, kw)}')
    return (n, h, wd, cin, cout, kh, kw, stride[0], stride[1], padding[0], padding[1], oh, ow)


def conv2d_fwd(x, w, b, stride, padding, pad_value=0.0, bias=True, act=None, alpha=0.0):
    dims = _conv_dims(x.shape, w.shape, stride, padding)
    code = _same_dtype(x, w, b)
    y = CP.empty((dims[0], dims[11], dims[12], dims[4]), x.dtype)
    _rt().call('uocr_conv2d_fwd', code, x.ptr, w.ptr, b.ptr, y.ptr, *dims, float(pad_value),
               int(bool(bias)), ACT_CODES[act], float(alpha))
    return y


def conv2d_bwd_data(dy, w, x_shape, stride, padding, x_act=None, act=None, alpha=0.0):
    dims = _conv_dims(x_shape, w.shape, stride, padding)
    code = _same_dtype(dy, w, grad=dy) if x_act is None else _same_dtype(dy, w, x_act, grad=dy)
    if dy.shape != (dims[0], dims[11], dims[12], dims[4]):
        raise AssertionError(f'grad shape {dy.shape} does not match the layer output')
    if x_act is not None and x_act.shape != tuple(x_shape):
        raise AssertionError(f'activation tensor {x_act.shape} != conv input {tuple(x_shape)}')
    dx = _like_grad(CP.empty(x_shape, dy.dtype), dy)
    _rt().call('uocr_conv2d_bwd_data', code, dy.ptr, w.ptr, dx.ptr, *dims,
               None if x_act is None else x_act.ptr, ACT_CODES[act if x_act is not None else None], float(alpha))
    return dx


def conv2d_bwd_weight(x, dy, dw, db, stride, padding, pad_value=0.0, bias=True, accumulate=True):
    dims = _conv_dims(x.shape, dw.shape, stride, padding)
    code = _same_dtype(x, dy, dw, db, grad=dy)
    with _rt().side(x, dy):
        _rt().call('uocr_conv2d_bwd_weight', code, x.ptr, dy.ptr, dw.ptr, db.ptr, *dims, float(pad_value),
                   int(bool(bias)), int(bool(accumulate)))
    _rt().keep(x, dy)


def conv_pair_fwd(x, w1, b1, w2, b2, pad_value1=0.0, bias1=True, bias2=True, alpha=0.01, act2=hiplib.ACT_NONE):
    n, h, wd, _ = x.shape
    code = _same_dtype(x, w1, b1, w2, b2)
    y = CP.empty((n, h, wd, 1), x.dtype)
    _rt().call('uocr_conv_pair_fwd', code, x.ptr, w1.ptr, b1.ptr, w2.ptr, b2.ptr, y.ptr, n, h, wd, w1.shape[3],
               float(pad_value1), int(bool(bias1)), int(bool(bias2)), float(alpha), int(act2))
    return y


def conv_pair_bwd(x, y, dy, w1, b1, w2, dw1, db1, dw2, db2, pad_value1=0.0, bias1=True, bias2=True, alpha=0.01,
                  act2=hiplib.ACT_NONE, need_dx=True, accumulate=True):
    n, h, wd, _ = x.shape
    code = _same_dtype(x, y, dy, w1, b1, w2, dw1, db1, dw2, db2, grad=dy)
    dx = _like_grad(CP.empty(x.shape, x.dtype), dy) if need_dx else None
    _rt().call('uocr_conv_pair_bwd', code, x.ptr, y.ptr, dy.ptr, w1.ptr, b1.ptr, w2.ptr, dw1.ptr, db1.ptr, dw2.ptr,
               db2.ptr, dx.ptr if need_dx else None, n, h, wd, w1.shape[3], float(pad_value1), int(bool(bias1)),
               int(bool(bias2)), float(alpha), int(act2), int(bool(accumulate)))
    return dx


def _up_dims(x_low_shape, w_shape, padding):
    n, hl, wl, cin = x_low_shape
    kh, kw, wcin, cout = w_shape
    assert wcin == cin
    return n, hl, wl, cin, cout, kh, kw, padding[0], padding[1]


def upconv2x_fwd(x_low, w, b, padding, bias=True, act=None, alpha=0.0, weff=None):
    dims = _up_dims(x_low.shape, w.shape, padding)
    code = _same_dtype(x_low, w, b)
    y = CP.empty((dims[0], 2 * dims[1], 2 * dims[2], dims[4]), x_low.dtype)
    _rt().call('uocr_upconv2x_fwd', code, x_low.ptr, w.ptr, b.ptr, y.ptr, *dims, int(bool(bias)), ACT_CODES[act],
               float(alpha), None if weff is None else weff.ptr)
    return y


def upconv2x_bwd_data(dy, w, x_low_shape, padding, x_act=None, act=None, alpha=0.0, weff=None):
    dims = _up_dims(x_low_shape, w.shape, padding)
    code = _same_dtype(dy, w, grad=dy)
    dx = _like_grad(CP.empty(x_low_shape, dy.dtype), dy)
    _rt().call('uocr_upconv2x_bwd_data', code, dy.ptr, w.ptr, dx.ptr, *dims, None if x_act is None else x_act.ptr,
               ACT_CODES[act if x_act is not None else None], float(alpha), None if weff is None else weff.ptr)
    return dx


def upconv2x_bwd_weight(x_low, dy, dw, db, padding, bias=True, accumulate=True):
    dims = _up_dims(x_low.shape, dw.shape, padding)
    code = _same_dtype(x_low, dy, dw, db, grad=dy)
    with _rt().side(x_low, dy):
        _rt().call('uocr_upconv2x_bwd_weight', code, x_low.ptr, dy.ptr, dw.ptr, db.ptr, *dims, int(bool(bias)),
                   int(bool(accumulate)))


def pool_out_hw(h, w, ks, stride, padding, ceil_mode):
    rnd = math.ceil if ceil_mode else math.floor
    return (rnd((h + 2 * padding[0] - (ks[0] - 1) - 1) / stride[0] + 1),
            rnd((w + 2 * padding[1] - (ks[1] - 1) - 1) / stride[1] + 1))


def maxpool2d_fwd(x, ks, stride, padding, ceil_mode=False):
    n, h, wd, c = x.shape
    oh, ow = pool_out_hw(h, wd, ks, stride, padding, ceil_mode)
    y = CP.empty((n, oh, ow, c), x.dtype)
    mask = CP.empty((n, ks[0] * oh, ks[1] * ow, c), np.uint8)
    _rt().call('uocr_maxpool2d_fwd', x.code, x.ptr, y.ptr, mask.ptr, n, h, wd, c, ks[0], ks[1], stride[0],
               stride[1], padding[0], padding[1], oh, ow)
    return y, mask


def maxpool2d_bwd(dy, mask, x_shape, ks, stride, padding):
    n, h, wd, c = x_shape
    oh, ow = dy.shape[1], dy.shape[2]
    dx = _like_grad(CP.empty(x_shape, dy.dtype), dy)
    _rt().call('uocr_maxpool2d_bwd', dy.code, dy.ptr, mask.ptr, dx.ptr, n, h, wd, c, ks[0], ks[1], stride[0],
               stride[1], padding[0], padding[1], oh, ow)
    return dx


def upsample2d_fwd(x, scale):
    n, h, wd, c = x.shape
    y = CP.empty((n, h * scale[0], wd * scale[1], c), x.dtype)
    _rt().call('uocr_upsample2d_fwd', x.code, x.ptr, y.ptr, n, h, wd, c, scale[0], scale[1])
    return y


def upsample2d_bwd(dy, x_shape, scale):
    n, h, wd, c = x_shape
    if dy.shape != (n, h * scale[0], wd * scale[1], c):
        raise AssertionError(f'grad shape {dy.shape} does not match the upsampled shape')
    dx = _like_grad(CP.empty(x_shape, dy.dtype), dy)
    _rt().call('uocr_upsample2d_bwd', dy.code, dy.ptr, dx.ptr, n, h, wd, c, scale[0], scale[1])
    return dx


def act_fwd(kind, x, alpha=0.0):
    y = CP.empty(x.shape, x.dtype)
    _rt().call('uocr_act_fwd', x.code, ACT_CODES[kind], float(alpha), x.ptr, y.ptr, x.size)
    return y


def act_bwd(kind, x, dy, alpha=0.0):
    code = _same_dtype(x, dy)
    if x.size != dy.size:
        raise AssertionError(f'grad size {dy.shape} != input size {x.shape}')
    dx = _like_grad(CP.empty(dy.shape, dy.dtype), dy)
    _rt().call('uocr_act_bwd', code, ACT_CODES[kind], float(alpha), x.ptr, dy.ptr, dx.ptr, x.size)
    return dx


def act_bwd_from_output(kind, y, dy, alpha=0.0):
    code = _same_dtype(y, dy)
    dx = _like_grad(CP.empty(dy.shape, dy.dtype), dy)
    _rt().call('uocr_act_bwd_from_output', code, ACT_CODES[kind], float(alpha), y.ptr, dy.ptr, dx.ptr, y.size)
    return dx


def dense_fwd(x, w, act=None, alpha=0.0):
    m, n_in = x.shape
    if w.shape[0] != n_in + 1:
        raise AssertionError(f'weights {w.shape} do not fit input {x.shape} (bias row included)')
    y = CP.empty((m, w.shape[1]), x.dtype)
    _rt().call('uocr_dense_fwd_act', _same_dtype(x, w), x.ptr, w.ptr, y.ptr, m, n_in, w.shape[1], ACT_CODES[act],
               float(alpha))
    return y


def dense_bwd(x, w, dy, dw, accumulate=True, need_dx=True, x_act=None, x_alpha=0.0):
    m, n_in = x.shape
    n_out = w.shape[1]
    code = _same_dtype(x, w, dy, dw, grad=dy)
    dx = _like_grad(CP.empty((m, n_in), dy.dtype), dy) if need_dx else None
    rt = _rt()
    if rt.side_on and need_dx:
        with rt.side(x, dy):
            rt.call('uocr_dense_bwd_act', code, x.ptr, w.ptr, dy.ptr, None, dw.ptr, m, n_in, n_out,
                    int(bool(accumulate)), ACT_CODES[None], 0.0)
        rt.call('uocr_dense_bwd_act', code, x.ptr, w.ptr, dy.ptr, dx.ptr, None, m, n_in, n_out, 0, ACT_CODES[x_act],
                float(x_alpha))
        return dx
    rt.call('uocr_dense_bwd_act', code, x.ptr, w.ptr, dy.ptr, dx.ptr if need_dx else None, dw.ptr, m, n_in,
            n_out, int(bool(accumulate)), ACT_CODES[x_act], float(x_alpha))
    rt.keep(x, dy)
    return dx


def _windows_dims(x_shape, w, width):
    n, h, wd, c = x_shape
    n_in = h * width * c
    if w.shape[0] != n_in + 1:
        raise AssertionError(f'weights {w.shape} do not fit {width}-column windows of {tuple(x_shape)} (bias row included)')
    if wd < width:
        raise AssertionError(f'Input width must be >= than output width, found: {wd} < {width}')
    dims = (n, h, wd, c, w.shape[1], h, width, 1, 1, 0, width // 2, 1, wd)
    return dims, n_in * w.shape[1] * w.t.element_size()


def windows_dense_fwd(x, w, width, act=None, alpha=0.0):
    dims, bias_off = _windows_dims(x.shape, w, width)
    y = CP.empty((dims[0] * dims[2], dims[4]), x.dtype)
    _rt().call('uocr_conv2d_fwd', _same_dtype(x, w), x.ptr, w.ptr, w.ptr + bias_off, y.ptr, *dims, 0.0, 1,
               ACT_CODES[act], float(alpha))
    return y


def windows_dense_bwd(x, w, dy, dw, width, accumulate=True, x_act=None, act=None, alpha=0.0):
    dims, bias_off = _windows_dims(x.shape, w, width)
    code = _same_dtype(x, w, dy, dw, grad=dy)
    if dy.shape != (dims[0] * dims[2], dims[4]):
        raise AssertionError(f'grad shape {dy.shape} does not match the layer output')
    with _rt().side(x, dy):
        _rt().call('uocr_conv2d_bwd_weight', code, x.ptr, dy.ptr, dw.ptr, dw.ptr + bias_off, *dims, 0.0, 1,
                   int(bool(accumulate)))
    _rt().keep(x, dy)
    dx = _like_grad(CP.empty(x.shape, dy.dtype), dy)
    _rt().call('uocr_conv2d_bwd_data', code, dy.ptr, w.ptr, dx.ptr, *dims, None if x_act is None else x_act.ptr,
               ACT_CODES[act if x_act is not None else None], float(alpha))
    return dx


def fixed_width_fwd(x, width):
    n, h, wd, c = x.shape
    y = CP.empty((n * wd, h, width, c), x.dtype)
    _rt().call('uocr_fixed_width_fwd', x.code, x.ptr, y.ptr, n, h, wd, c, width)
    return y


def fixed_width_bwd(dy, x_shape, width):
    n, h, wd, c = x_shape
    dx = _like_grad(CP.empty(x_shape, dy.dtype), dy)
    _rt().call('uocr_fixed_width_bwd', dy.code, dy.ptr, dx.ptr, n, h, wd, c, width)
    return dx


def concat(arrays, axis=-1):
    nd = arrays[0].ndim
    axis = axis % nd
    lead = arrays[0].shape[:axis]
    rows = int(np.prod(lead)) if lead else 1
    tails = [int(np.prod(a.shape[axis:])) for a in arrays]
    out_shape = list(arrays[0].shape)
    out_shape[axis] = sum(a.shape[axis] for a in arrays)
    out = CP.empty(out_shape, arrays[0].dtype)
    total = sum(tails)
    off = 0
    esz = out.t.element_size()
    for a, cols in zip(arrays, tails):
        _same_dtype(out, a)
        _rt().call('uocr_copy_2d', out.code, out.ptr + off * esz, total, a.ptr, cols, rows, cols)
        off += cols
    return out


def split(array, shapes, axis=-1):
    nd = array.ndim
    axis = axis % nd
    rows = int(np.prod(array.shape[:axis])) if axis else 1
    total = int(np.prod(array.shape[axis:]))
    outs, off = [], 0
    esz = array.t.element_size()
    for shp in shapes:
        cols = int(np.prod(shp[axis:]))
        out = _like_grad(CP.empty(shp, array.dtype), array)
        _rt().call('uocr_copy_2d', out.code, out.ptr, cols, array.ptr + off * esz, total, rows, cols)
        outs.append(out)
        off += cols
    return outs


def add(a, b):
    if a.shape != b.shape:
        raise AssertionError(f'cannot add {a.shape} and {b.shape}')
    if a.gscale != b.gscale:
        raise HipError(f'cannot add gradients that carry different scales (2^{a.gscale} and 2^{b.gscale})')
    out = _like_grad(CP.empty(a.shape, a.dtype), a)
    _rt().call('uocr_add', _same_dtype(a, b), a.ptr, b.ptr, out.ptr, a.size)
    return out


def axpy(alpha, x, y):
    _rt().call('uocr_axpy', _same_dtype(x, y), float(alpha), x.ptr, y.ptr, x.size)


def scale_(x, alpha):
    _rt().call('uocr_scale', x.code, float(alpha), x.ptr, x.size)


def fill_(x, value):
    _rt().call('uocr_fill', x.code, x.ptr, float(value), x.size)


def zero_(x):
    _rt().call('uocr_memset_zero', x.ptr, x.nbytes)


def u8_to_float(src_u8, scale=1.0 / 255.0, dtype=None, out=None):
    if out is None:
        out = CP.empty(src_u8.shape, CP.dtype if dtype is None else dtype)
    elif out.shape != src_u8.shape:
        raise AssertionError(f'u8_to_float: out {out.shape} != source {src_u8.shape}')
    _rt().call('uocr_u8_to_float', out.code, src_u8.ptr, out.ptr, float(scale), out.size)
    return out


def _loss_slot():
    return CP.loss_slot()


def _loss_code(pred, gt, grad, kind, n):
    code = _same_dtype(pred, gt)
    if code == hiplib.F16 and grad is not None:
        grad.gscale = f16_grad_scale_log2(kind, n)
        return hiplib.f16_scaled(grad.gscale)
    return code


def _finish_loss(slot):
    return DeviceScalar(slot.t) if CP.lazy_losses else float(slot.t.item())


def seg_loss(kind, pred, gt, need_grad=True, out_act=None):
    n, h, w, c = pred.shape
    if gt.shape != pred.shape:
        raise AssertionError(f'ground truth {gt.shape} != prediction {pred.shape}')
    grad = CP.empty(pred.shape, pred.dtype) if need_grad else None
    slot = _loss_slot()
    _rt().call('uocr_seg_loss', _loss_code(pred, gt, grad, 'seg', h * w), hiplib.LOSS_DICE if kind == 'dice' else hiplib.LOSS_JACCARD,
               pred.ptr, gt.ptr, grad.ptr if need_grad else None, slot.ptr, n, h * w, c, ACT_CODES[out_act])
    return _finish_loss(slot), grad


def softmax_ce(pred, gt, need_grad=True):
    m, c = pred.shape
    if gt.shape != pred.shape:
        raise AssertionError(f'ground truth {gt.shape} != prediction {pred.shape}')
    grad = CP.empty(pred.shape, pred.dtype) if need_grad else None
    slot = _loss_slot()
    _rt().call('uocr_softmax_ce', _loss_code(pred, gt, grad, 'ce', m), pred.ptr, gt.ptr, grad.ptr if need_grad else None,
               slot.ptr, m, c)
    return _finish_loss(slot), grad


def sigmoid_ce(pred, gt, need_grad=True):
    if gt.shape != pred.shape:
        raise AssertionError(f'ground truth {gt.shape} != prediction {pred.shape}')
    grad = CP.empty(pred.shape, pred.dtype) if need_grad else None
    slot = _loss_slot()
    _rt().call('uocr_sigmoid_ce', _loss_code(pred, gt, grad, 'ce', gt.shape[0]), pred.ptr, gt.ptr, grad.ptr if need_grad else None,
               slot.ptr, gt.shape[0], pred.size)
    return _finish_loss(slot), grad


def regularize(kind, w, grad, strength, slot=None, accumulate=False):
    own = slot is None
    if own:
        slot = _loss_slot()
    _rt().call('uocr_l2_reg' if kind == 'l2' else 'uocr_l1_reg', _same_dtype(w, grad), w.ptr, grad.ptr, w.size,
               float(strength), slot.ptr, int(bool(accumulate)))
    return _finish_loss(slot) if own else None


def adam_step(w, g, v, a, lr, beta1, beta2, eps):
    _rt().call('uocr_adam_step', _same_dtype(w, g, v, a), w.ptr, g.ptr, v.ptr, a.ptr, w.size, float(lr),
               float(beta1), float(beta2), float(eps))


def _range_args(ranges):
    import ctypes as C
    n = len(ranges)
    lo = (C.c_longlong * max(n, 1))(*[r[1] for r in ranges])
    hi = (C.c_longlong * max(n, 1))(*[r[2] for r in ranges])
    kind = (C.c_int * max(n, 1))(*[{'l1': 1, 'l2': 2, 1: 1, 2: 2}[r[0][0]] for r in ranges])
    strength = (C.c_double * max(n, 1))(*[float(r[0][1]) for r in ranges])
    return n, lo, hi, kind, strength


def momentum_step_fused(w, g, v, lr, momentum, ranges, zero_grad=True, hyper=None):
    n, lo, hi, kind, strength = _range_args(ranges)
    slot = _loss_slot() if n else None
    _rt().call('uocr_momentum_step_fused', _same_dtype(w, g, v), w.ptr, g.ptr, v.ptr, w.size, float(lr), float(momentum),
               n, lo, hi, kind, strength, slot.ptr if n else None, int(bool(zero_grad)),
               None if hyper is None else hyper.ptr)
    return _finish_loss(slot) if n else 0


def adam_step_fused(w, g, v, a, lr, beta1, beta2, eps, ranges, zero_grad=True, hyper=None):
    n, lo, hi, kind, strength = _range_args(ranges)
    slot = _loss_slot() if n else None
    _rt().call('uocr_adam_step_fused', _same_dtype(w, g, v, a), w.ptr, g.ptr, v.ptr, a.ptr, w.size, float(lr),
               float(beta1), float(beta2), float(eps), n, lo, hi, kind, strength, slot.ptr if n else None,
               int(bool(zero_grad)), None if hyper is None else hyper.ptr)
    return _finish_loss(slot) if n else 0


def momentum_step(w, g, v, lr, momentum):
    _rt().call('uocr_momentum_step', _same_dtype(w, g, v), w.ptr, g.ptr, v.ptr, w.size, float(lr), float(momentum))


def rmsprop_step(w, g, a, lr, rho, eps):
    _rt().call('uocr_rmsprop_step', _same_dtype(w, g, a), w.ptr, g.ptr, a.ptr, w.size, float(lr), float(rho),
               float(eps))


def has_nan(x):
    flag = CP.empty((1,), np.int32)
    _rt().call('uocr_has_nan', x.code, x.ptr, x.size, flag.ptr)
    return bool(flag.t.item())


class _Ops:
    add = staticmethod(add)


CP.ops = _Ops
```

Measured before the change: 32320 images/s.

## Fuse upconv2x weight and data gradients into one warp-specialized backward kernel

Adds a combined upconv2x backward entry point and kernel with 512 threads per block. Half the threads compute the data gradient with FMA, and the other half accumulate the weight gradient with MFMA. Both halves share one staged copy of the x_low and dy tiles in shared memory. This removes a second kernel launch and a duplicate read of dy and x. The Python layer uses it only when the side stream is off, so with multi-queue settings the old two-op path may still run, and the larger block may lower occupancy.

```diff
diff --git a/include/univer_hip.h b/include/univer_hip.h
--- a/include/univer_hip.h
+++ b/include/univer_hip.h
@@ -95,6 +95,9 @@
 int uocr_upconv2x_bwd_weight(uocr_ctx* ctx, int dtype, const void* x_low, const void* dy, void* dw, void* db,
                              int n, int hl, int wl, int cin, int cout, int kh, int kw, int ph, int pw,
                              int use_bias, int accumulate);
+int uocr_upconv2x_bwd(uocr_ctx* ctx, int dtype, const void* x_low, const void* dy, const void* w, void* dx_low,
+                      void* dw, void* db, int n, int hl, int wl, int cin, int cout, int kh, int kw, int ph, int pw,
+                      const void* x_act, int act, double act_alpha, const void* weff, int use_bias, int accumulate);
 
 int uocr_maxpool2d_fwd(uocr_ctx* ctx, int dtype, const void* x, void* y, uint8_t* mask,
                        int n, int h, int wd, int c, int kh, int kw, int sh, int sw, int ph, int pw,
diff --git a/univer-ocr_amd/csrc/conv_up.hip b/univer-ocr_amd/csrc/conv_up.hip
--- a/univer-ocr_amd/csrc/conv_up.hip
+++ b/univer-ocr_amd/csrc/conv_up.hip
@@ -48,11 +48,11 @@
     }
 }
 
-template <typename TA>
+template <int NT = 256, typename TA>
 __device__ __forceinline__ void stage_planar(float* __restrict__ xs, const TA* __restrict__ xb, int ry, int rx,
                                              int hl, int wl, int tid) {
     if constexpr (sizeof(TA) == 4) {
-        stage_batched<XH * XW, 256, 3, float4>(
+        stage_batched<XH * XW, NT, (XH * XW + NT - 1) / NT, float4>(
             tid,
             [&](int i, bool& inside) {
                 const int r = i / XW, c = i - r * XW;
@@ -69,7 +69,7 @@
             });
         return;
     }
-    for (int i = tid; i < XH * XW; i += 256) {
+    for (int i = tid; i < XH * XW; i += NT) {
         const int r = i / XW, c = i - r * XW;
         const int gy = ry - 1 + r, gx = rx - 1 + c;
         float4 v = make_float4(0.f, 0.f, 0.f, 0.f);
@@ -142,6 +142,62 @@
     }
 }
 
+template <typename G>
+__device__ __forceinline__ void up4_wgrad_tile(const float* __restrict__ xs, int wv, int kq, const int (&aoff)[3],
+                                               const bool (&aok)[3], f32x4 (&acc)[3], float& dbacc, G g_at) {
+#pragma unroll 2
+    for (int k = 0; k < 8; ++k) {
+        const int gi = wv * 8 + k, r = gi >> 1, c0 = (gi & 1) * 16;
+        const float* xr = xs + r * XW + c0;
+#pragma unroll
+        for (int i = 0; i < 4; ++i) {
+            const float g = g_at(r, c0 + 4 * i + kq);
+            dbacc += g;
+#pragma unroll
+            for (int j = 0; j < 3; ++j) {
+                const float xv = xr[4 * i + aoff[j]];
+                acc[j] = mfma(aok[j] ? xv : 0.f, g, acc[j]);
+            }
+        }
+    }
+}
+
+__device__ __forceinline__ void up4_wgrad_aoff(int n, int kq, int (&aoff)[3], bool (&aok)[3]) {
+#pragma unroll
+    for (int j = 0; j < 3; ++j) {
+        const int K = 16 * j + n;
+        aok[j] = K < 36;
+        const int Kc = aok[j] ? K : 35, t = Kc >> 2;
+        aoff[j] = (Kc & 3) * XPLANE + (t / 3) * XW + t % 3 + kq;
+    }
+}
+
+__device__ __forceinline__ void up4_wgrad_row(float (*red)[48][16], float (*reddb)[64], const f32x4 (&acc)[3], float dbacc,
+                                              float* __restrict__ partial, int tid, int nthreads, bool owner) {
+    const int lane = tid & 63, wv = (tid >> 6) & 3, n = lane & 15, kq = lane >> 4;
+    if (owner) {
+#pragma unroll
+        for (int j = 0; j < 3; ++j)
+#pragma unroll
+            for (int v = 0; v < 4; ++v) red[wv][16 * j + 4 * kq + v][n] = acc[j][v];
+        reddb[wv][lane] = dbacc;
+    }
+    __syncthreads();
+    if (tid < 4) {
+        float s = 0.f;
+        for (int w = 0; w < 4; ++w)
+            for (int l = tid; l < 64; l += 4) s += reddb[w][l];
+        reddb[0][tid] = s;
+    }
+    __syncthreads();
+    const int blk = (blockIdx.z * gridDim.y + blockIdx.y) * gridDim.x + blockIdx.x;
+    up4_write_row(partial + (size_t)blk * UP4_NOUT, [&](int i) {
+        if (i >= 576) return reddb[0][i - 576];
+        const int K = i >> 4, col = i & 15;
+        return red[0][K][col] + red[1][K][col] + red[2][K][col] + red[3][K][col];
+    }, tid, nthreads);
+}
+
 template <typename TA>
 __global__ __launch_bounds__(256) void upconv_wgrad_kernel(const TA* __restrict__ xl, const TA* __restrict__ dy,
                                                            float* __restrict__ partial, int hl, int wl,
@@ -157,13 +213,7 @@
     const TA* gb = dy + (size_t)blockIdx.z * (2 * hl) * W * CH;
     int aoff[3];
     bool aok[3];
-#pragma unroll
-    for (int j = 0; j < 3; ++j) {
-        const int K = 16 * j + n;
-        aok[j] = K < 36;
-        const int Kc = aok[j] ? K : 35, t = Kc >> 2;
-        aoff[j] = (Kc & 3) * XPLANE + (t / 3) * XW + t % 3 + kq;
-    }
+    up4_wgrad_aoff(n, kq, aoff, aok);
     const int boff = ((n >> 3) * W + ((n >> 2) & 1)) * CH + (n & 3);
     f32x4 acc[3] = {{0.f, 0.f, 0.f, 0.f}, {0.f, 0.f, 0.f, 0.f}, {0.f, 0.f, 0.f, 0.f}};
     float dbacc = 0.f;
@@ -171,47 +221,14 @@
         __syncthreads();
         stage_planar(xs, xb, ry, rx, hl, wl, tid);
         __syncthreads();
-#pragma unroll 2
-        for (int k = 0; k < 8; ++k) {
-            const int gi = wv * 8 + k, r = gi >> 1, c0 = (gi & 1) * 16;
+        up4_wgrad_tile(xs, wv, kq, aoff, aok, acc, dbacc, [&](int r, int pl) {
             const int py = ry + r;
-            const bool row_ok = py < row_end;
-            const float* xr = xs + r * XW + c0;
-            const TA* gr = gb + ((size_t)(2 * min(py, hl - 1)) * W + 2 * rx) * CH + boff;
-#pragma unroll
-            for (int i = 0; i < 4; ++i) {
-                const int pl = c0 + 4 * i + kq;
-                const bool ok = row_ok && rx + pl < wl;
-                float g = ld1(gr + (size_t)2 * min(pl, wl - 1 - rx) * CH);
-                g = ok ? g : 0.f;
-                dbacc += g;
-#pragma unroll
-                for (int j = 0; j < 3; ++j) {
-                    const float xv = xr[4 * i + aoff[j]];
-                    acc[j] = mfma(aok[j] ? xv : 0.f, g, acc[j]);
-                }
-            }
-        }
-    }
-#pragma unroll
-    for (int j = 0; j < 3; ++j)
-#pragma unroll
-        for (int v = 0; v < 4; ++v) red[wv][16 * j + 4 * kq + v][n] = acc[j][v];
-    reddb[wv][lane] = dbacc;
-    __syncthreads();
-    if (tid < 4) {
-        float s = 0.f;
-        for (int w = 0; w < 4; ++w)
-            for (int l = tid; l < 64; l += 4) s += reddb[w][l];
-        reddb[0][tid] = s;
-    }
-    __syncthreads();
-    const int blk = (blockIdx.z * gridDim.y + blockIdx.y) * gridDim.x + blockIdx.x;
-    up4_write_row(partial + (size_t)blk * UP4_NOUT, [&](int i) {
-        if (i >= 576) return reddb[0][i - 576];
-        const int K = i >> 4, col = i & 15;
-        return red[0][K][col] + red[1][K][col] + red[2][K][col] + red[3][K][col];
-    }, tid, 256);
+            const bool ok = py < row_end && rx + pl < wl;
+            const float g = ld1(gb + ((size_t)(2 * min(py, hl - 1)) * W + 2 * rx) * CH + boff + (size_t)2 * min(pl, wl - 1 - rx) * CH);
+            return ok ? g : 0.f;
+        });
+    }
+    up4_wgrad_row(red, reddb, acc, dbacc, partial, tid, 256, true);
 }
 
 __global__ __launch_bounds__(256) void colsum_finish_kernel(const float* __restrict__ partial, int nblocks, int ncols,
@@ -245,6 +262,76 @@
 }
 
 constexpr int GH = 2 * (RH + 2), GW = 2 * (RW + 2);
+
+template <int NT = 256, typename TA>
+__device__ __forceinline__ void stage_dy4(float4* __restrict__ gs, const TA* __restrict__ gb, int ry, int rx, int H, int W,
+                                          int tid) {
+    if constexpr (sizeof(TA) == 4) {
+        stage_batched<GH * GW, NT, 5, float4>(
+            tid,
+            [&](int i, bool& inside) {
+                const int r = i / GW, c = i - r * GW;
+                const int gy = 2 * (ry - 1) + r, gx = 2 * (rx - 1) + c;
+                inside = gy >= 0 && gy < H && gx >= 0 && gx < W;
+                return reinterpret_cast<const float4*>(gb + ((size_t)min(max(gy, 0), H - 1) * W + min(max(gx, 0), W - 1)) * CH);
+            },
+            [&](int i, float4 v, bool inside) { gs[i] = inside ? v : make_float4(0.f, 0.f, 0.f, 0.f); });
+    } else {
+        for (int i = tid; i < GH * GW; i += NT) {
+            const int r = i / GW, c = i - r * GW;
+            const int gy = 2 * (ry - 1) + r, gx = 2 * (rx - 1) + c;
+            float4 v = make_float4(0.f, 0.f, 0.f, 0.f);
+            if (gy >= 0 && gy < H && gx >= 0 && gx < W) v = ld4(gb + ((size_t)gy * W + gx) * CH);
+            gs[i] = v;
+        }
+    }
+}
+
+template <typename TA, typename M>
+__device__ __forceinline__ void up4_dgrad_tile(const float4* __restrict__ gs, const float* __restrict__ weff,
+                                               TA* __restrict__ dxl, int img, int ry, int rx, int hl, int wl, int tid,
+                                               int mask_act, float mask_alpha, M act_out) {
+    const int c = tid & 31, r0 = tid >> 5;
+    float acc[2][4];
+#pragma unroll
+    for (int p = 0; p < 2; ++p)
+#pragma unroll
+        for (int j = 0; j < 4; ++j) acc[p][j] = 0.f;
+#pragma unroll 1
+    for (int m = 0; m < 9; ++m) {
+        const float* wt = weff + m * 64;
+        const int my = m / 3 - 1, mx = m % 3 - 1;
+#pragma unroll
+        for (int p = 0; p < 2; ++p) {
+            const int r = r0 + 8 * p;
+            const float4* g0 = gs + (2 * (r - my + 1)) * GW + 2 * (c - mx + 1);
+            const float4 g[4] = {g0[0], g0[1], g0[GW], g0[GW + 1]};
+#pragma unroll
+            for (int ch = 0; ch < 4; ++ch)
+#pragma unroll
+                for (int phase = 0; phase < 4; ++phase) {
+                    const float* wv = wt + ch * 16 + phase * 4;
+                    acc[p][ch] += wv[0] * g[phase].x + wv[1] * g[phase].y + wv[2] * g[phase].z + wv[3] * g[phase].w;
+                }
+        }
+    }
+#pragma unroll
+    for (int p = 0; p < 2; ++p) {
+        const int qy = ry + r0 + 8 * p, qx = rx + c;
+        if (qy >= hl || qx >= wl) continue;
+        const size_t off = (((size_t)img * hl + qy) * wl + qx) * CH;
+        float4 out = make_float4(acc[p][0], acc[p][1], acc[p][2], acc[p][3]);
+        if (mask_act != UOCR_ACT_NONE) {
+            const float4 yv = act_out(p, off);
+            out.x *= act_grad_from_output<float>(yv.x, mask_act, mask_alpha);
+            out.y *= act_grad_from_output<float>(yv.y, mask_act, mask_alpha);
+            out.z *= act_grad_from_output<float>(yv.z, mask_act, mask_alpha);
+            out.w *= act_grad_from_output<float>(yv.w, mask_act, mask_alpha);
+        }
+        st4(dxl + off, out);
+    }
+}
+
 template <typename TA>
 __global__ __launch_bounds__(256) void upconv_dgrad_kernel(const TA* __restrict__ dy, const float* __restrict__ weff,
                                                            TA* __restrict__ dxl, int hl, int wl,
@@ -254,66 +341,52 @@
     const int tid = threadIdx.x;
     const int rx = blockIdx.x * RW, ry = blockIdx.y * RH;
     const int H = 2 * hl, W = 2 * wl;
+    stage_dy4(gs, dy + (size_t)blockIdx.z * H * W * CH, ry, rx, H, W, tid);
+    __syncthreads();
+    up4_dgrad_tile(gs, weff, dxl, blockIdx.z, ry, rx, hl, wl, tid, mask_act, mask_alpha,
+                   [&](int, size_t off) { return ld4(mask_y + off); });
+}
+
+constexpr int BWD_NT = 512;
+template <typename TA>
+__global__ __launch_bounds__(BWD_NT, 4) void upconv_bwd_kernel(const TA* __restrict__ xl, const TA* __restrict__ dy,
+                                                               const float* __restrict__ weff, TA* __restrict__ dxl,
+                                                               float* __restrict__ partial, int hl, int wl,
+                                                               int rows_per_block, int mask_act, float mask_alpha) {
+    __shared__ float4 gs[GH * GW];
+    __shared__ float xs[CH * XPLANE];
+    static_assert(sizeof(float) * (4 * 48 * 16 + 4 * 64) <= sizeof(float4) * GH * GW, "the reduction arrays alias the dy tile");
+    float (*red)[48][16] = reinterpret_cast<float (*)[48][16]>(gs);
+    float (*reddb)[64] = reinterpret_cast<float (*)[64]>(reinterpret_cast<float*>(gs) + 4 * 48 * 16);
+    const int tid = threadIdx.x, lane = tid & 63, n = lane & 15, kq = lane >> 4;
+    const bool mma = tid >= 256;
+    const int t2 = tid & 255, wv = t2 >> 6;
+    const int rx = blockIdx.x * RW;
+    const int row_begin = blockIdx.y * rows_per_block, row_end = min(hl, row_begin + rows_per_block);
+    const int H = 2 * hl, W = 2 * wl;
+    const TA* xb = xl + (size_t)blockIdx.z * hl * wl * CH;
     const TA* gb = dy + (size_t)blockIdx.z * H * W * CH;
-    if constexpr (sizeof(TA) == 4) {
-        stage_batched<GH * GW, 256, 5, float4>(
-            tid,
-            [&](int i, bool& inside) {
-                const int r = i / GW, c = i - r * GW;
-                const int gy = 2 * (ry - 1) + r, gx = 2 * (rx - 1) + c;
-                inside = gy >= 0 && gy < H && gx >= 0 && gx < W;
-                return reinterpret_cast<const float4*>(gb + ((size_t)min(max(gy, 0), H - 1) * W + min(max(gx, 0), W - 1)) * CH);
-            },
-            [&](int i, float4 v, bool inside) { gs[i] = inside ? v : make_float4(0.f, 0.f, 0.f, 0.f); });
-    } else {
-        for (int i = tid; i < GH * GW; i += 256) {
-            const int r = i / GW, c = i - r * GW;
-            const int gy = 2 * (ry - 1) + r, gx = 2 * (rx - 1) + c;
-            float4 v = make_float4(0.f, 0.f, 0.f, 0.f);
-            if (gy >= 0 && gy < H && gx >= 0 && gx < W) v = ld4(gb + ((size_t)gy * W + gx) * CH);
-            gs[i] = v;
-        }
+    int aoff[3];
+    bool aok[3];
+    up4_wgrad_aoff(n, kq, aoff, aok);
+    const float* gsb = reinterpret_cast<const float*>(gs) + ((2 + (n >> 3)) * GW + 2 + ((n >> 2) & 1)) * CH + (n & 3);
+    f32x4 acc[3] = {{0.f, 0.f, 0.f, 0.f}, {0.f, 0.f, 0.f, 0.f}, {0.f, 0.f, 0.f, 0.f}};
+    float dbacc = 0.f;
+    for (int ry = row_begin; ry < row_end; ry += RH) {
+        __syncthreads();
+        stage_planar<BWD_NT>(xs, xb, ry, rx, hl, wl, tid);
+        stage_dy4<BWD_NT>(gs, gb, ry, rx, H, W, tid);
+        __syncthreads();
+        if (!mma)
+            up4_dgrad_tile(gs, weff, dxl, blockIdx.z, ry, rx, hl, wl, t2, mask_act, mask_alpha, [&](int p, size_t) {
+                const float* xc = xs + ((t2 >> 5) + 8 * p + 1) * XW + (t2 & 31) + 1;
+                return make_float4(xc[0], xc[XPLANE], xc[2 * XPLANE], xc[3 * XPLANE]);
+            });
+        else
+            up4_wgrad_tile(xs, wv, kq, aoff, aok, acc, dbacc, [&](int r, int pl) { return gsb[(2 * r * GW + 2 * pl) * CH]; });
     }
     __syncthreads();
-    const int c = tid & 31, r0 = tid >> 5;
-    float acc[2][4];
-#pragma unroll
-    for (int p = 0; p < 2; ++p)
-#pragma unroll
-        for (int j = 0; j < 4; ++j) acc[p][j] = 0.f;
-#pragma unroll 1
-    for (int m = 0; m < 9; ++m) {
-        const float* wt = weff + m * 64;
-        const int my = m / 3 - 1, mx = m % 3 - 1;
-#pragma unroll
-        for (int p = 0; p < 2; ++p) {
-            const int r = r0 + 8 * p;
-            const float4* g0 = gs + (2 * (r - my + 1)) * GW + 2 * (c - mx + 1);
-            const float4 g[4] = {g0[0], g0[1], g0[GW], g0[GW + 1]};
-#pragma unroll
-            for (int ch = 0; ch < 4; ++ch)
-#pragma unroll
-                for (int phase = 0; phase < 4; ++phase) {
-                    const float* wv = wt + ch * 16 + phase * 4;
-                    acc[p][ch] += wv[0] * g[phase].x + wv[1] * g[phase].y + wv[2] * g[phase].z + wv[3] * g[phase].w;
-                }
-        }
-    }
-#pragma unroll
-    for (int p = 0; p < 2; ++p) {
-        const int qy = ry + r0 + 8 * p, qx = rx + c;
-        if (qy >= hl || qx >= wl) continue;
-        const size_t off = (((size_t)blockIdx.z * hl + qy) * wl + qx) * CH;
-        float4 out = make_float4(acc[p][0], acc[p][1], acc[p][2], acc[p][3]);
-        if (mask_act != UOCR_ACT_NONE) {
-            const float4 yv = ld4(mask_y + off);
-            out.x *= act_grad_from_output<float>(yv.x, mask_act, mask_alpha);
-            out.y *= act_grad_from_output<float>(yv.y, mask_act, mask_alpha);
-            out.z *= act_grad_from_output<float>(yv.z, mask_act, mask_alpha);
-            out.w *= act_grad_from_output<float>(yv.w, mask_act, mask_alpha);
-        }
-        st4(dxl + off, out);
-    }
+    up4_wgrad_row(red, reddb, acc, dbacc, partial, tid, BWD_NT, mma);
 }
 
 __device__ __forceinline__ void weff1_build(float (&we)[36], const float* __restrict__ w) {
@@ -373,6 +446,57 @@
     }
 }
 
+template <int NT = 256, typename TA>
+__device__ __forceinline__ void stage_x1(float* __restrict__ xs, const TA* __restrict__ xb, int ry, int rx, int hl, int wl,
+                                         int tid) {
+    stage_batched<XH * XW, NT, (XH * XW + NT - 1) / NT, TA>(
+        tid,
+        [&](int i, bool& inside) {
+            const int r = i / XW, cc = i - r * XW;
+            const int gy = ry - 1 + r, gx = rx - 1 + cc;
+            inside = gy >= 0 && gy < hl && gx >= 0 && gx < wl;
+            return xb + (size_t)min(max(gy, 0), hl - 1) * wl + min(max(gx, 0), wl - 1);
+        },
+        [&](int i, TA v, bool inside) { xs[i] = inside ? (float)v : 0.f; });
+}
+
+template <int NT = 256, typename TA>
+__device__ __forceinline__ void stage_dy1(float* __restrict__ gs, const TA* __restrict__ gb, int ry, int rx, int H, int W,
+                                          int tid) {
+    stage_batched<GH * GW, NT, (GH * GW + NT - 1) / NT, TA>(
+        tid,
+        [&](int i, bool& inside) {
+            const int r = i / GW, c = i - r * GW;
+            const int gy = 2 * (ry - 1) + r, gx = 2 * (rx - 1) + c;
+            inside = gy >= 0 && gy < H && gx >= 0 && gx < W;
+            return gb + (size_t)min(max(gy, 0), H - 1) * W + min(max(gx, 0), W - 1);
+        },
+        [&](int i, TA v, bool inside) { gs[i] = inside ? (float)v : 0.f; });
+}
+
+template <typename TA, typename M>
+__device__ __forceinline__ void up1_dgrad_tile(const float* __restrict__ gs, const float (&we)[36], TA* __restrict__ dxl,
+                                               int img, int ry, int rx, int hl, int wl, int tid, int mask_act,
+                                               float mask_alpha, M act_out) {
+    const int c = tid & 31, r0 = tid >> 5;
+#pragma unroll
+    for (int p = 0; p < 2; ++p) {
+        const int r = r0 + 8 * p;
+        float acc = 0.f;
+#pragma unroll
+        for (int m = 0; m < 9; ++m) {
+            const int my = m / 3 - 1, mx = m % 3 - 1;
+            const float* g0 = gs + (2 * (r - my + 1)) * GW + 2 * (c - mx + 1);
+            acc += we[m * 4] * g0[0] + we[m * 4 + 1] * g0[1] + we[m * 4 + 2] * g0[GW] + we[m * 4 + 3] * g0[GW + 1];
+        }
+        const int qy = ry + r, qx = rx + c;
+        if (qy >= hl || qx >= wl) continue;
+        const size_t off = ((size_t)img * hl + qy) * wl + qx;
+        if (mask_act != UOCR_ACT_NONE) acc *= act_grad_from_output<float>(act_out(r, off), mask_act, mask_alpha);
+        st1(dxl + off, acc);
+    }
+}
+
 template <typename TA>
 __global__ __launch_bounds__(256) void up1_dgrad_kernel(const TA* __restrict__ dy, const float* __restrict__ w,
                                                         TA* __restrict__ dxl, int hl, int wl,
@@ -382,36 +506,40 @@
     const int tid = threadIdx.x;
     const int rx = blockIdx.x * RW, ry = blockIdx.y * RH;
     const int H = 2 * hl, W = 2 * wl;
-    const TA* gb = dy + (size_t)blockIdx.z * H * W;
-    stage_batched<GH * GW, 256, 10, TA>(
-        tid,
-        [&](int i, bool& inside) {
-            const int r = i / GW, c = i - r * GW;
-            const int gy = 2 * (ry - 1) + r, gx = 2 * (rx - 1) + c;
-            inside = gy >= 0 && gy < H && gx >= 0 && gx < W;
-            return gb + (size_t)min(max(gy, 0), H - 1) * W + min(max(gx, 0), W - 1);
-        },
-        [&](int i, TA v, bool inside) { gs[i] = inside ? (float)v : 0.f; });
+    stage_dy1(gs, dy + (size_t)blockIdx.z * H * W, ry, rx, H, W, tid);
     float we[36];
     weff1_build(we, w);
     __syncthreads();
-    const int c = tid & 31, r0 = tid >> 5;
-#pragma unroll
-    for (int p = 0; p < 2; ++p) {
-        const int r = r0 + 8 * p;
-        float acc = 0.f;
-#pragma unroll
-        for (int m = 0; m < 9; ++m) {
-            const int my = m / 3 - 1, mx = m % 3 - 1;
-            const float* g0 = gs + (2 * (r - my + 1)) * GW + 2 * (c - mx + 1);
-            acc += we[m * 4] * g0[0] + we[m * 4 + 1] * g0[1] + we[m * 4 + 2] * g0[GW] + we[m * 4 + 3] * g0[GW + 1];
-        }
-        const int qy = ry + r, qx = rx + c;
-        if (qy >= hl || qx >= wl) continue;
-        const size_t off = ((size_t)blockIdx.z * hl + qy) * wl + qx;
-        if (mask_act != UOCR_ACT_NONE) acc *= act_grad_from_output<float>(ld1(mask_y + off), mask_act, mask_alpha);
-        st1(dxl + off, acc);
-    }
+    up1_dgrad_tile(gs, we, dxl, blockIdx.z, ry, rx, hl, wl, tid, mask_act, mask_alpha,
+                   [&](int, size_t off) { return ld1(mask_y + off); });
+}
+
+__device__ __forceinline__ void up1_wgrad_pos(const float* __restrict__ xs, int r, int c, const float (&g)[4],
+                                              float (&acc)[36], float& dbacc) {
+    dbacc += (g[0] + g[1]) + (g[2] + g[3]);
+#pragma unroll
+    for (int m = 0; m < 9; ++m) {
+        const float xv = xs[(r + m / 3) * XW + c + m % 3];
+#pragma unroll
+        for (int phase = 0; phase < 4; ++phase) acc[m * 4 + phase] += xv * g[phase];
+    }
+}
+
+__device__ __forceinline__ void up1_wgrad_row(float (*red)[37], const float (&acc)[36], float dbacc,
+                                              float* __restrict__ partial, int tid, bool owner) {
+    const int lane = tid & 63, wv = (tid >> 6) & 3;
+    if (owner) {
+#pragma unroll
+        for (int i = 0; i < 36; ++i) {
+            const float v = wave_reduce_sum(acc[i]);
+            if (lane == 0) red[wv][i] = v;
+        }
+        dbacc = wave_reduce_sum(dbacc);
+        if (lane == 0) red[wv][36] = dbacc;
+    }
+    __syncthreads();
+    const int blk = (blockIdx.z * gridDim.y + blockIdx.y) * gridDim.x + blockIdx.x;
+    up1_write_row(partial + (size_t)blk * UP1_NOUT, [&](int i) { return red[0][i] + red[1][i] + red[2][i] + red[3][i]; }, tid);
 }
 
 template <typename TA>
@@ -432,15 +560,7 @@
     for (int i = 0; i < 36; ++i) acc[i] = 0.f;
     for (int ry = row_begin; ry < row_end; ry += RH) {
         __syncthreads();
-        stage_batched<XH * XW, 256, 3, TA>(
-            tid,
-            [&](int i, bool& inside) {
-                const int r = i / XW, cc = i - r * XW;
-                const int gy = ry - 1 + r, gx = rx - 1 + cc;
-                inside = gy >= 0 && gy < hl && gx >= 0 && gx < wl;
-                return xb + (size_t)min(max(gy, 0), hl - 1) * wl + min(max(gx, 0), wl - 1);
-            },
-            [&](int i, TA v, bool inside) { xs[i] = inside ? (float)v : 0.f; });
+        stage_x1(xs, xb, ry, rx, hl, wl, tid);
         __syncthreads();
 #pragma unroll
         for (int p = 0; p < 2; ++p) {
@@ -449,26 +569,53 @@
             const TA* g0 = gb + (size_t)(2 * py) * W + 2 * pxl;
             const float2 ga = ld2(g0), gbv = ld2(g0 + W);
             const float g[4] = {ga.x, ga.y, gbv.x, gbv.y};
-            dbacc += (g[0] + g[1]) + (g[2] + g[3]);
-#pragma unroll
-            for (int m = 0; m < 9; ++m) {
-                const float xv = xs[(r + m / 3) * XW + c + m % 3];
-#pragma unroll
-                for (int phase = 0; phase < 4; ++phase) acc[m * 4 + phase] += xv * g[phase];
+            up1_wgrad_pos(xs, r, c, g, acc, dbacc);
+        }
+    }
+    up1_wgrad_row(red, acc, dbacc, partial, tid, true);
+}
+
+template <typename TA>
+__global__ __launch_bounds__(BWD_NT, 4) void up1_bwd_kernel(const TA* __restrict__ xl, const TA* __restrict__ dy,
+                                                            const float* __restrict__ w, TA* __restrict__ dxl,
+                                                            float* __restrict__ partial, int hl, int wl,
+                                                            int rows_per_block, int mask_act, float mask_alpha) {
+    __shared__ float gs[GH * GW];
+    __shared__ float xs[XH * XW];
+    __shared__ float red[4][37];
+    const int tid = threadIdx.x, t2 = tid & 255;
+    const bool sums = tid >= 256;
+    const int rx = blockIdx.x * RW;
+    const int row_begin = blockIdx.y * rows_per_block, row_end = min(hl, row_begin + rows_per_block);
+    const int H = 2 * hl, W = 2 * wl;
+    const TA* xb = xl + (size_t)blockIdx.z * hl * wl;
+    const TA* gb = dy + (size_t)blockIdx.z * H * W;
+    const int c = t2 & 31, r0 = t2 >> 5;
+    float acc[36], dbacc = 0.f;
+#pragma unroll
+    for (int i = 0; i < 36; ++i) acc[i] = 0.f;
+    for (int ry = row_begin; ry < row_end; ry += RH) {
+        __syncthreads();
+        stage_x1<BWD_NT>(xs, xb, ry, rx, hl, wl, tid);
+        stage_dy1<BWD_NT>(gs, gb, ry, rx, H, W, tid);
+        __syncthreads();
+        if (!sums) {
+            float we[36];
+            weff1_build(we, w);
+            up1_dgrad_tile(gs, we, dxl, blockIdx.z, ry, rx, hl, wl, t2, mask_act, mask_alpha,
+                           [&](int r, size_t) { return xs[(r + 1) * XW + c + 1]; });
+        } else {
+#pragma unroll
+            for (int p = 0; p < 2; ++p) {
+                const int r = r0 + 8 * p;
+                if (ry + r >= row_end || rx + c >= wl) continue;
+                const float* g0 = gs + (2 * (r + 1)) * GW + 2 * (c + 1);
+                const float g[4] = {g0[0], g0[1], g0[GW], g0[GW + 1]};
+                up1_wgrad_pos(xs, r, c, g, acc, dbacc);
             }
         }
     }
-    const int lane = tid & 63, wv = tid >> 6;
-#pragma unroll
-    for (int i = 0; i < 36; ++i) {
-        const float v = wave_reduce_sum(acc[i]);
-        if (lane == 0) red[wv][i] = v;
-    }
-    dbacc = wave_reduce_sum(dbacc);
-    if (lane == 0) red[wv][36] = dbacc;
-    __syncthreads();
-    const int blk = (blockIdx.z * gridDim.y + blockIdx.y) * gridDim.x + blockIdx.x;
-    up1_write_row(partial + (size_t)blk * UP1_NOUT, [&](int i) { return red[0][i] + red[1][i] + red[2][i] + red[3][i]; }, tid);
+    up1_wgrad_row(red, acc, dbacc, partial, tid, sums);
 }
 
 
@@ -486,6 +633,25 @@
                   "upconv2x: 5x5 / padding 2 / 4 -> 4 or 1 -> 1 channels only (got %dx%d pad %d,%d %d -> %d)", kh, kw, ph,
                   pw, cin, cout);
     UOCR_REQUIRE(ctx, n > 0 && hl > 0 && wl > 0 && n <= 65535);
+    return UOCR_OK;
+}
+
+int up_finish(uocr_ctx* ctx, const float* partial, int nblocks, int ncols, int ndw, void* dw, void* db, int use_bias,
+              int accumulate, float unscale) {
+    FinishDesc fd{};
+    fd.kind = FIN_COLS;
+    fd.partial = partial;
+    fd.nblocks = nblocks;
+    fd.ncols = fd.group_cols = ncols;
+    fd.row_stride = ncols;
+    fd.dw = (float*)dw, fd.db = (float*)db;
+    fd.use_bias = use_bias, fd.accumulate = accumulate;
+    fd.unscale = unscale;
+    fd.p[0] = ndw;
+    if (uocr_finish_defer(ctx, fd)) return UOCR_OK;
+    hipLaunchKernelGGL(colsum_finish_kernel, dim3((ncols + 7) / 8), dim3(256), 0, ctx->stream, partial, nblocks, ncols,
+                       ndw, (float*)dw, (float*)db, use_bias, accumulate, unscale);
+    UOCR_LAUNCH_CHECK(ctx);
     return UOCR_OK;
 }
 
@@ -559,23 +725,6 @@
     if (rc != UOCR_OK) return rc;
     const float unscale = (float)uocr_grad_unscale(dtype);
     const int ncols = cin == 1 ? UP1_NOUT : UP4_NOUT, ndw = ncols - cin;
-    auto finish = [&](const float* partial, int nblocks) -> int {
-        FinishDesc fd{};
-        fd.kind = FIN_COLS;
-        fd.partial = partial;
-        fd.nblocks = nblocks;
-        fd.ncols = fd.group_cols = ncols;
-        fd.row_stride = ncols;
-        fd.dw = (float*)dw, fd.db = (float*)db;
-        fd.use_bias = use_bias, fd.accumulate = accumulate;
-        fd.unscale = unscale;
-        fd.p[0] = ndw;
-        if (uocr_finish_defer(ctx, fd)) return UOCR_OK;
-        hipLaunchKernelGGL(colsum_finish_kernel, dim3((ncols + 7) / 8), dim3(256), 0, ctx->stream, partial, nblocks, ncols,
-                           ndw, (float*)dw, (float*)db, use_bias, accumulate, unscale);
-        UOCR_LAUNCH_CHECK(ctx);
-        return UOCR_OK;
-    };
     if (UOCR_DTYPE_BASE(dtype) == UOCR_F16 && ctx->opt_fast && ctx->opt_h16 && uocr_aligned_act(x_low, dtype) &&
         uocr_aligned_act(dy, dtype)) {
         const size_t floats = (size_t)ctx->cu_count * 8 * ncols;
@@ -584,7 +733,7 @@
         int nblocks = 0;
         rc = uocr_upconv_wgrad_h16(ctx, x_low, dy, partial, floats, n, hl, wl, cin, &nblocks);
         if (rc != UOCR_OK) return rc;
-        return finish(partial, nblocks);
+        return up_finish(ctx, partial, nblocks, ncols, ndw, dw, db, use_bias, accumulate, unscale);
     }
     const int strips = (wl + RW - 1) / RW, rows = up_rows_per_block(strips, hl, n, (unsigned)uocr_budget(ctx, 1024));
     const int bands = (hl + rows - 1) / rows, nblocks = strips * bands * n;
@@ -600,5 +749,45 @@
                                (const TA*)x_low, (const TA*)dy, partial, hl, wl, rows);
     });
     UOCR_LAUNCH_CHECK(ctx);
-    return finish(partial, nblocks);
-}
+    return up_finish(ctx, partial, nblocks, ncols, ndw, dw, db, use_bias, accumulate, unscale);
+}
+
+extern "C" int uocr_upconv2x_bwd(uocr_ctx* ctx, int dtype, const void* x_low, const void* dy, const void* w, void* dx_low,
+                                 void* dw, void* db, int n, int hl, int wl, int cin, int cout, int kh, int kw, int ph, int pw,
+                                 const void* x_act, int act, double act_alpha, const void* weff_in, int use_bias,
+                                 int accumulate) {
+    UOCR_CHECK_CTX(ctx);
+    UOCR_REQUIRE(ctx, x_low && dy && w && dx_low && dw && db);
+    UOCR_REQUIRE(ctx, act == UOCR_ACT_NONE || x_act != nullptr);
+    int rc = check_up(ctx, dtype, n, hl, wl, cin, cout, kh, kw, ph, pw);
+    if (rc != UOCR_OK) return rc;
+    if (!ctx->opt_up_bwd || dtype != UOCR_F32 || uocr_upconv_t32_eligible(ctx, dtype, cin, cout) ||
+        (act != UOCR_ACT_NONE && x_act != x_low)) {
+        rc = uocr_upconv2x_bwd_weight(ctx, dtype, x_low, dy, dw, db, n, hl, wl, cin, cout, kh, kw, ph, pw, use_bias, accumulate);
+        if (rc != UOCR_OK) return rc;
+        return uocr_upconv2x_bwd_data(ctx, dtype, dy, w, dx_low, n, hl, wl, cin, cout, kh, kw, ph, pw, x_act, act, act_alpha,
+                                      weff_in);
+    }
+    const int ncols = cin == 1 ? UP1_NOUT : UP4_NOUT, ndw = ncols - cin;
+    const int strips = (wl + RW - 1) / RW, rows = up_rows_per_block(strips, hl, n, (unsigned)uocr_budget(ctx, 1024));
+    const int bands = (hl + rows - 1) / rows, nblocks = strips * bands * n;
+    uocr_note_split(ctx, nblocks, (long long)strips * ((hl + RH - 1) / RH) * n);
+    const size_t nrows = ((size_t)nblocks * ncols + 3) & ~(size_t)3;
+    const bool make_weff = cin != 1 && !weff_in;
+    float* partial = uocr_partial_buffer(ctx, (nrows + (make_weff ? NWEFF : 0)) * sizeof(float), &rc);
+    if (rc != UOCR_OK) return rc;
+    const float* weff = (const float*)weff_in;
+    if (make_weff) {
+        hipLaunchKernelGGL(upconv_weff_kernel, dim3(1), dim3(256), 0, ctx->stream, (const float*)w, partial + nrows);
+        weff = partial + nrows;
+    }
+    if (cin == 1)
+        hipLaunchKernelGGL((up1_bwd_kernel<float>), dim3(strips, bands, n), dim3(BWD_NT), 0, ctx->stream, (const float*)x_low,
+                           (const float*)dy, (const float*)w, (float*)dx_low, partial, hl, wl, rows, act, (float)act_alpha);
+    else
+        hipLaunchKernelGGL((upconv_bwd_kernel<float>), dim3(strips, bands, n), dim3(BWD_NT), 0, ctx->stream,
+                           (const float*)x_low, (const float*)dy, weff, (float*)dx_low, partial, hl, wl, rows, act,
+                           (float)act_alpha);
+    UOCR_LAUNCH_CHECK(ctx);
+    return up_finish(ctx, partial, nblocks, ncols, ndw, dw, db, use_bias, accumulate, (float)uocr_grad_unscale(dtype));
+}
diff --git a/univer-ocr_amd/csrc/ctx.hip b/univer-ocr_amd/csrc/ctx.hip
--- a/univer-ocr_amd/csrc/ctx.hip
+++ b/univer-ocr_amd/csrc/ctx.hip
@@ -42,6 +42,7 @@
     ctx->opt_group_blocks = 0;
     ctx->opt_wgrad_bands = 0;
     ctx->opt_max_blocks = 0;
+    ctx->opt_up_bwd = 1;
     ctx->split_blocks = 0;
     ctx->split_items = 0;
     ctx->gemm_bm = ctx->gemm_gm = ctx->gemm_gn = ctx->gemm_nsplit = 0;
@@ -147,6 +148,7 @@
     else if (!strcmp(key, "group_blocks")) ctx->opt_group_blocks = value;
     else if (!strcmp(key, "wgrad_bands") && value >= 0) ctx->opt_wgrad_bands = value;
     else if (!strcmp(key, "max_blocks") && value >= 0) ctx->opt_max_blocks = value;
+    else if (!strcmp(key, "up_bwd")) ctx->opt_up_bwd = value;
     else if (!strcmp(key, "h3")) {
 #ifndef UOCR_EXPERIMENTS
         if (value) UOCR_FAIL(ctx, UOCR_ERR_UNSUPPORTED, "option h3: this library was built without conv_h3 "
diff --git a/univer-ocr_amd/csrc/uocr_common.h b/univer-ocr_amd/csrc/uocr_common.h
--- a/univer-ocr_amd/csrc/uocr_common.h
+++ b/univer-ocr_amd/csrc/uocr_common.h
@@ -36,6 +36,7 @@
     int opt_group_blocks;
     int opt_wgrad_bands;
     int opt_pair_g;
+    int opt_up_bwd;
     int opt_max_blocks;
     int split_blocks;
     long long split_items;
diff --git a/univer-ocr_amd/hip/lib.py b/univer-ocr_amd/hip/lib.py
--- a/univer-ocr_amd/hip/lib.py
+++ b/univer-ocr_amd/hip/lib.py
@@ -77,6 +77,7 @@
     'uocr_upconv2x_fwd': [_ctx, _i, _vp, _vp, _vp, _vp] + [_i] * 9 + [_i, _i, _d, _vp],
     'uocr_upconv2x_bwd_data': [_ctx, _i, _vp, _vp, _vp] + [_i] * 9 + [_vp, _i, _d, _vp],
     'uocr_upconv2x_bwd_weight': [_ctx, _i, _vp, _vp, _vp, _vp] + [_i] * 9 + [_i, _i],
+    'uocr_upconv2x_bwd': [_ctx, _i, _vp, _vp, _vp, _vp, _vp, _vp] + [_i] * 9 + [_vp, _i, _d, _vp, _i, _i],
     'uocr_maxpool2d_fwd': [_ctx, _i, _vp, _vp, _vp] + [_i] * 12,
     'uocr_maxpool2d_bwd': [_ctx, _i, _vp, _vp, _vp] + [_i] * 12,
     'uocr_upsample2d_fwd': [_ctx, _i, _vp, _vp] + [_i] * 6,
diff --git a/univer-ocr_amd/nn/layers/convolutional.py b/univer-ocr_amd/nn/layers/convolutional.py
--- a/univer-ocr_amd/nn/layers/convolutional.py
+++ b/univer-ocr_amd/nn/layers/convolutional.py
@@ -110,14 +110,16 @@
         if activation is not None and not act_grad_applied:
             grad = ops.act_bwd_from_output(activation.kind, self._fused_out, grad, activation.alpha)
         x_low = self._mem[0]
-        ops.upconv2x_bwd_weight(x_low, grad, self.w.grad, self.b.grad, self.padding, self.bias, accumulate=True)
         weff = getattr(self, '_weff', None)
         self._weff = None
-        if input_activation is None:
-            dx = ops.upconv2x_bwd_data(grad, self.w.value, x_low.shape, self.padding, weff=weff)
+        mask = {} if input_activation is None else dict(x_act=x_low, act=input_activation.kind,
+                                                        alpha=input_activation.alpha)
+        if CP.runtime().side_on:
+            ops.upconv2x_bwd_weight(x_low, grad, self.w.grad, self.b.grad, self.padding, self.bias, accumulate=True)
+            dx = ops.upconv2x_bwd_data(grad, self.w.value, x_low.shape, self.padding, weff=weff, **mask)
         else:
-            dx = ops.upconv2x_bwd_data(grad, self.w.value, x_low.shape, self.padding, x_act=x_low,
-                                       act=input_activation.kind, alpha=input_activation.alpha, weff=weff)
+            dx = ops.upconv2x_bwd(x_low, grad, self.w.value, self.w.grad, self.b.grad, self.padding, self.bias,
+                                  accumulate=True, weff=weff, **mask)
         self._fused_out = None
         self.clear_memory()
         return dx
diff --git a/univer-ocr_amd/nn/ops.py b/univer-ocr_amd/nn/ops.py
--- a/univer-ocr_amd/nn/ops.py
+++ b/univer-ocr_amd/nn/ops.py
@@ -142,6 +142,16 @@
     with _rt().side(x_low, dy):
         _rt().call('uocr_upconv2x_bwd_weight', code, x_low.ptr, dy.ptr, dw.ptr, db.ptr, *dims, int(bool(bias)),
                    int(bool(accumulate)))
+
+
+def upconv2x_bwd(x_low, dy, w, dw, db, padding, bias=True, accumulate=True, x_act=None, act=None, alpha=0.0, weff=None):
+    dims = _up_dims(x_low.shape, w.shape, padding)
+    code = _same_dtype(x_low, dy, w, dw, db, grad=dy)
+    dx = _like_grad(CP.empty(x_low.shape, dy.dtype), dy)
+    _rt().call('uocr_upconv2x_bwd', code, x_low.ptr, dy.ptr, w.ptr, dx.ptr, dw.ptr, db.ptr, *dims,
+               None if x_act is None else x_act.ptr, ACT_CODES[act if x_act is not None else None], float(alpha),
+               None if weff is None else weff.ptr, int(bool(bias)), int(bool(accumulate)))
+    return dx
 
 
 def pool_out_hw(h, w, ks, stride, padding, ceil_mode):
```

Measured after the change: 31980 images/s. -1.0%, worse.
